# cv-core/MIT-Driverless-CV-TrainingInfra

Measured on AMD Instinct MI355X. Metric: images/sec training (YOLOv3 416^2 + RektNet 80^2), higher is better.
Workload: dtype bf16; 1 GPU; CVC-YOLOv3 yolo_baseline 416x416 classes=80, train step (fwd+bwd+Adam), 32 img/GPU; global_batch=32, parallelism=dp1, hipgraph=False, optimizer=FusedAdam

## Files before the change

include/mdcv_hip.h:

```cpp
#ifndef MDCV_HIP_H
#define MDCV_HIP_H
#ifdef __cplusplus
extern "C" {
#endif

#define MDCV_OK 0
#define MDCV_EARG (-1)
#define MDCV_F32 0
#define MDCV_BF16 1
#define MDCV_TUNED(dtype, code) (((dtype) & 0xff) | ((code) * 256))
#define MDCV_ACT_NONE 0
#define MDCV_ACT_LEAKY 1
#define MDCV_ACT_RELU 2

int mdcv_conv2d(int dtype, int mode, const void* in, int in_ldc, const void* w_packed, void* out, int out_ldc,
                const float* bias, const void* addsrc, int add_ldc, float* stats_partial,
                int B, int Hin, int Win, int Cin, int Hout, int Wout, int Nout,
                int KH, int KW, int stride, int pad, int dil, void* stream);
int mdcv_conv2d_affine_act(int dtype, const void* in, int in_ldc, const void* w_packed, void* out, int out_ldc, const float* scale,
                           const float* shift, const void* addsrc, int add_ldc, int act, float slope, int B, int Hin, int Win, int Cin,
                           int Hout, int Wout, int Nout, int KH, int KW, int stride, int pad, int dil, void* stream);
int mdcv_conv2d_dgrad_bnsums_rows(int dtype, int B, int Hin, int Win, int Cin, int Hout, int Wout, int Nout, int KH, int KW, int stride,
                                  int pad, int dil, int in_ldc);
int mdcv_conv2d_dgrad_bnsums(int dtype, const void* in, int in_ldc, const void* w_packed, void* out, int out_ldc, const void* addsrc,
                             int add_ldc, int B, int Hin, int Win, int Cin, int Hout, int Wout, int Nout, int KH, int KW, int stride,
                             int pad, int dil, const void* y, int ldy, const float* scale, const float* shift, const float* mean, int act,
                             float slope, float* partial, void* stream);
int mdcv_first_conv_ok(int dtype, int B, int H, int W, int Cin_pad, int Cout_pad, int KH, int KW, int stride, int pad, int dil, int ldx);
int mdcv_first_conv_rows(int B, int H);
int mdcv_first_conv_stats(int dtype, const void* x, int ldx, const void* w_packed, float* partial, int B, int H, int W, void* stream);
int mdcv_first_conv_bn_act(int dtype, const void* x, int ldx, const void* w_packed, const float* scale, const float* shift, int act, float slope,
                           void* y, int ldy, void* z, int ldz, int B, int H, int W, void* stream);
int mdcv_conv2d_dgrad_s2_form_ok(int dtype, int B, int Hin, int Win, int Cin, int Hout, int Wout, int Nout, int KH, int KW, int stride,
                                 int pad, int dil, int in_ldc);
int mdcv_xstats_words(int reps, int C);
int mdcv_xstats_reps(int rows, int C);
int mdcv_conv2d_xstats(int dtype, const void* in, int in_ldc, const void* w_packed, void* out, int out_ldc, const float* bias, void* xacc,
                       int reps, int B, int Hin, int Win, int Cin, int Hout, int Wout, int Nout, int KH, int KW, int stride, int pad, int dil,
                       void* stream);
int mdcv_pw_conv_fwd_xstats(int dtype, const void* y, int ldy, const float* scale, const float* shift, const void* resid, int ldr, int act,
                            float slope, void* z_out, int ldz, const void* w_packed, const float* bias, void* out, int out_ldc, void* xacc,
                            int reps, long long M, int K, int N, void* stream);
int mdcv_bn_act_fwd_xstats(int dtype, const void* y, int ldy, const void* xacc, int reps, double count, const float* gamma, const float* beta,
                           float* running_mean, float* running_var, float momentum, float eps, float* scale, float* shift, float* mean,
                           float* invstd, const void* resid, int ldr, void* out, int ldo, int M, int C, int act, float slope, void* stream);
int mdcv_conv2d_stats_rows(int M);
int mdcv_conv2d_stats_rows_geom(int dtype, int B, int Hout, int Wout, int Cin, int Nout, int KH, int KW, int stride, int pad, int dil,
                                int in_ldc);

int mdcv_conv2d_wgrad_splits(int dtype, int M, int Cout, int Ktot);
int mdcv_conv2d_wgrad_splits_geom(int dtype, int B, int Hin, int Win, int Cin, int Hout, int Wout, int Cout, int KH, int KW, int stride,
                                  int pad, int dil, int dy_ldc, int x_ldc);
int mdcv_conv2d_wgrad(int dtype, const void* dy, int dy_ldc, const void* x, int x_ldc, float* ws, int splits,
                      float* dw_oihw, int accumulate, int B, int Hin, int Win, int Cin, int Cin_real,
                      int Hout, int Wout, int Cout, int Cout_real, int KH, int KW, int stride, int pad, int dil, void* stream);

int mdcv_pack_weights(int dtype, const float* w_oihw, void* w_fwd, void* w_dgrad, int Cout, int Cin, int KH, int KW,
                      int Cout_pad, int Cin_pad, void* stream);

int mdcv_pack_weights_batched(int dtype, const void* table, int nlayers, int max_taps, void* stream);

int mdcv_nchw_to_nhwc(int dtype, const float* src, void* dst, int B, int C, int H, int W, int ldc, int Cpad, void* stream);
int mdcv_nhwc_to_nchw(int dtype, const void* src, int ldc, float* dst, int B, int C, int H, int W, void* stream);

int mdcv_partial_reduce(const float* partial, int rows, int nsums, int C, double* accum, void* stream);
int mdcv_bn_finalize(double* accum, double count, const float* gamma, const float* beta, float* running_mean, float* running_var,
                     float momentum, float eps, float* scale, float* shift, float* mean, float* invstd, int C, void* stream);
int mdcv_bn_eval_coeffs(const float* gamma, const float* beta, const float* running_mean, const float* running_var, float eps,
                        float* scale, float* shift, int C, void* stream);
int mdcv_bn_eval_coeffs_bias(const float* gamma, const float* beta, const float* running_mean, const float* running_var, float eps,
                             const float* conv_bias, float* scale, float* shift, int C, void* stream);
int mdcv_bn_act_fwd(int dtype, const void* y1, int ld1, const float* s1, const float* b1, const void* y2, int ld2, const float* s2,
                    const float* b2, const void* resid, int ldr, void* out, int ldo, int M, int C, int act, float slope, void* stream);
int mdcv_bn_act_bwd_reduce_ws_floats(int dtype, int M, int C, int nsums);
int mdcv_bn_stats_finalize(const float* partial, int rows, double* accum, double count, const float* gamma, const float* beta,
                           float* running_mean, float* running_var, float momentum, float eps, float* scale, float* shift, float* mean,
                           float* invstd, int C, void* stream);
int mdcv_bn_act_bwd_reduce_finalize(int dtype, const void* dout, int ldd, const void* y1, int ld1, const float* s1, const float* b1,
                                    const float* mean1, const float* invstd1, const void* y2, int ld2, const float* s2, const float* b2,
                                    const float* mean2, const float* invstd2, float* partial_ws, int M, int C, int act, float slope,
                                    double count, const float* gamma1, float* dgamma1, float* dbeta1, float* cA1, float* cB1, float* cC1,
                                    const float* gamma2, float* dgamma2, float* dbeta2, float* cA2, float* cB2, float* cC2, void* stream);
int mdcv_bn_bwd_finalize_rows(const float* partial, int rows, int C, double count, const float* gamma, const float* mean,
                              const float* invstd, float* dgamma, float* dbeta, float* cA, float* cB, float* cC, void* stream);
int mdcv_bn_act_bwd_reduce(int dtype, const void* dout, int ldd, const void* y1, int ld1, const float* s1, const float* b1,
                           const float* mean1, const float* invstd1, const void* y2, int ld2, const float* s2, const float* b2,
                           const float* mean2, const float* invstd2, double* accum, float* partial_ws, int M, int C, int act, float slope,
                           void* stream);
int mdcv_bn_bwd_finalize(double* accum, int kx, int nsums, int zero_after, double count, const float* gamma, const float* mean,
                         const float* invstd, float* dgamma, float* dbeta, float* cA, float* cB, float* cC, int C, void* stream);
int mdcv_bn_act_bwd_apply(int dtype, const void* dout, int ldd, const void* y1, int ld1, const float* s1, const float* b1,
                          const float* cA1, const float* cB1, const float* cC1, void* dy1, int ldy1,
                          const void* y2, int ld2, const float* s2, const float* b2, const float* cA2, const float* cB2,
                          const float* cC2, void* dy2, int ldy2, int M, int C, int act, float slope, void* stream);
int mdcv_colsum(int dtype, const void* x, int ldc, int M, int C, double* accum, void* stream);
int mdcv_colsum_ws_floats(int dtype, int M, int C);
int mdcv_colsum_f32(int dtype, const void* x, int ldc, int M, int C, float* partial_ws, float* out, void* stream);
int mdcv_accum_to_f32(double* accum, float* out, int n, int zero_after, void* stream);

int mdcv_upsample2x_fwd(int dtype, const void* in, int ldi, void* out, int ldo, int B, int H, int W, int C, void* stream);
int mdcv_upsample2x_bwd(int dtype, const void* dout, int ldo, void* din, int ldi, int B, int H, int W, int C, void* stream);

int mdcv_maxpool2x2_fwd(int dtype, const void* in, int ldi, void* out, int ldo, unsigned char* idx, int B, int H, int W, int C, int stride,
                        void* stream);
int mdcv_maxpool2x2_bwd(int dtype, const void* dout, int ldo, const unsigned char* idx, void* din, int ldi, int B, int H, int W, int C, int stride,
                        void* stream);

int mdcv_maxpool_fwd(int dtype, const void* in, int ldi, void* out, int ldo, unsigned char* idx, int B, int H, int W, int C, int k, int stride,
                     int pad, void* stream);
int mdcv_maxpool_bwd(int dtype, const void* dout, int ldo, const unsigned char* idx, void* din, int ldi, int B, int H, int W, int C, int k, int stride,
                     int pad, void* stream);
int mdcv_upsample_fwd(int dtype, const void* in, int ldi, void* out, int ldo, int B, int H, int W, int C, int scale, void* stream);
int mdcv_upsample_bwd(int dtype, const void* dout, int ldo, void* din, int ldi, int B, int H, int W, int C, int scale, void* stream);

long long mdcv_yolo_head_workspace_bytes(int B, int A, int Gh, int Gw);
int mdcv_yolo_head_train(int dtype, const void* logits, int ldc, void* dlogits, int ldd, int Cpad, const float* targets,
                         const float* anchors_scaled, int B, int T, int A, int C, int Gh, int Gw, float thresh, float xy_loss,
                         float wh_loss, float obj_loss, float noobj_loss, void* workspace, float* out7, const float* gscale,
                         void* stream);
int mdcv_yolo_head_grad(int dtype, const void* logits, int ldc, void* dlogits, int ldd, int Cpad, const float* targets,
                        const float* anchors_scaled, int B, int T, int A, int C, int Gh, int Gw, float thresh, float xy_loss,
                        float wh_loss, float obj_loss, float noobj_loss, void* workspace, const float* gscale, void* stream);
int mdcv_yolo_head_decode(int dtype, const void* logits, int ldc, const float* anchors_scaled, float stride, int B, int A, int C, int Gh,
                          int Gw, float* out, int rows_total, int row_off, void* stream);
int mdcv_bbox_iou(const float* box1, long long n1, int stride1, const float* box2, long long n2, int stride2, int corners, float* out, void* stream);
long long mdcv_build_targets_workspace_bytes(int B, int T, int A, int Gh, int Gw);
int mdcv_build_targets(const float* targets, const float* anchors, int B, int T, int A, int C, int Gh, int Gw, float thresh,
                       unsigned char* mask, unsigned char* conf_mask, float* tx, float* ty, float* tw, float* th, float* tconf,
                       unsigned char* tcls, void* workspace, int* err_out, void* stream);

int mdcv_head1x1_f32(const void* x_bf16, int ldx, const float* w, const float* bias, float* out, long long M, int C, int K, void* stream);
int mdcv_softargmax_fwd(int dtype, const void* logits, int ldc, int B, int K, int H, int W, float* hm, float* pts, void* stream);
int mdcv_softargmax_bwd(int dtype, const float* hm, const float* pts, const float* dpts, const float* dhm, float* sdot_ws, int B, int K,
                        int H, int W, void* dlogits, int ldd, void* stream);
int mdcv_cross_ratio_loss(const float* hm, const float* pts, const float* thm, const float* tpts, int B, int H, int W, int loss_type,
                          int include_geo, float gamma_horz, float gamma_vert, double* acc_ws, const float* gscale, float* out3,
                          float* dpts, float* dhm, void* stream);

#define MDCV_KPT_EVAL_ROW 12
int mdcv_kpt_eval_rows(const float* hm, const float* pts, const float* thm, const float* tpts, int B, int H, int W, int loss_type, int include_geo,
                       float gamma_horz, float gamma_vert, float dist_sx, float dist_sy, float* rows, void* stream);

#define MDCV_NMS_MAX_TOPK 512
long long mdcv_nms_workspace_bytes(int n);
int mdcv_nms(const float* boxes, const float* scores, int n, float overlap, int top_k, long long* keep, int* count, void* workspace,
             void* stream);
long long mdcv_detect_post_workspace_bytes(int B, int N);
int mdcv_detect_post(const float* pred, int B, int N, int C, const float* targets, int T, float conf_thres, float nms_thres,
                     float iou_thres, float width, float height, int top_k, float* out_boxes, float* out_prob, int* out_cls,
                     long long* out_index, unsigned char* out_correct, int* out_count, float* out_stats, void* workspace,
                     void* stream);
int mdcv_average_precision(const unsigned char* tp, const float* conf, int m, int n_gt, float* out3, void* stream);

int mdcv_crop_resize(const float* frames, int B, int C, int H, int W, const float* boxes, const int* count, int K, float scale_x,
                     float scale_y, float off_x, float off_y, int out_h, int out_w, float* out, int* owner, int* total, void* stream);

int mdcv_crop_resize_u8(const unsigned char* frames, int B, int C, int H, int W, const float* boxes, const int* count, int K, float scale_x,
                        float scale_y, float off_x, float off_y, int out_h, int out_w, float* out, int* owner, int* total, void* stream);

int mdcv_synth_cone_batch(unsigned int seed, int step, int B, int T, int H, int W, int num_classes, float* images, float* targets, void* stream);
int mdcv_synth_crop_batch(unsigned int seed, int step, int B, int size, float* images, float* heatmaps, float* points, void* stream);

#define MDCV_IMGLOAD_DESC 20
long long mdcv_imgload_workspace_bytes(int B, int max_scr_w, int max_scr_h);
int mdcv_imgload_batch(const int* desc_host, const int* desc, int B, const int* coefs, long long n_coefs, const unsigned char* src,
                       long long src_bytes, int max_scr_w, int max_scr_h, int C, int H, int W, void* workspace, float* out, void* stream);

#define MDCV_IMGAUG_DESC 24
long long mdcv_imgaug_workspace_bytes(int B, int H, int W);
int mdcv_imgload_aug_batch(const int* desc_host, const int* desc, const int* aug_host, const int* aug, int B, const int* coefs, long long n_coefs,
                           const unsigned char* src, long long src_bytes, int max_scr_w, int max_scr_h, int C, int H, int W, void* workspace,
                           void* aug_workspace, float* out, void* stream);

#define MDCV_IMGLOAD_FREF 4
int mdcv_imgload_frames_batch(const int* desc_host, const int* desc, const long long* fref_host, const long long* fref, int B, const int* coefs,
                              long long n_coefs, const unsigned char* src, long long src_bytes, const unsigned char* pool, long long pool_bytes,
                              int max_scr_w, int max_scr_h, int C, int H, int W, void* workspace, float* out, void* stream);
int mdcv_imgload_aug_frames_batch(const int* desc_host, const int* desc, const long long* fref_host, const long long* fref, const int* aug_host,
                                  const int* aug, int B, const int* coefs, long long n_coefs, const unsigned char* src, long long src_bytes,
                                  const unsigned char* pool, long long pool_bytes, int max_scr_w, int max_scr_h, int C, int H, int W,
                                  void* workspace, void* aug_workspace, float* out, void* stream);

#define MDCV_IMGFX_DESC 24
int mdcv_imgfx_batch(const int* fx_host, const int* fx, int B, const unsigned char* luts, int n_luts, int C, int H, int W, const float* src,
                     float* dst, void* stream);

#define MDCV_KPTLOAD_DESC 20
#define MDCV_KPTLOAD_MIN_SIZE 16
#define MDCV_KPTLOAD_MAX_SIZE 256
#define MDCV_KPTLOAD_MAX_SIDE 4096
int mdcv_kptload_batch(const int* desc_host, const int* desc, int B, const unsigned char* src, long long src_bytes, int S, float* images,
                       float* heatmaps, void* stream);

#define MDCV_DETECT_DESC 6
int mdcv_detect_draw_boxes(const long long* desc_host, const long long* desc, int B, const float* boxes, const int* count, int K,
                           unsigned char* pool, long long pool_bytes, int red, int green, int blue, double* frame_boxes, int* rects,
                           int* skipped, void* stream);

int mdcv_detect_map_boxes(const long long* desc_host, const long long* desc, int B, const float* boxes, const int* count, int K,
                          long long pool_bytes, double* frame_boxes, int* rects, int* skipped, void* stream);

int mdcv_crop_resize_frames_u8(const long long* desc_host, const long long* desc, int B, const unsigned char* pool, long long pool_bytes,
                               const int* rects, const int* count, int K, int max_per_frame, int S, float* crops, int* owner, int* window,
                               int* total, void* stream);
int mdcv_kpt_draw_points(const long long* desc_host, const long long* desc, int n_images, unsigned char* pool, long long pool_bytes,
                         const float* pts, const int* window, const int* owner, int M, const unsigned char* colours, int* centers,
                         int* skipped, void* stream);
int mdcv_kpt_heatmap_mosaic(const float* hm, int B, int S, unsigned char* out, void* stream);

int mdcv_adam_step(float* params, const float* grads, float* exp_avg, float* exp_avg_sq, long long n, int step, float lr, float beta1,
                   float beta2, float eps, float weight_decay, float grad_scale, void* stream);
int mdcv_sgd_step(float* params, const float* grads, float* momentum_buf, long long n, int step, float lr, float momentum, float weight_decay,
                  float grad_scale, void* stream);

int mdcv_device_info(int* cu_count, int* wave_size, long long* hbm_bytes, char* arch, int arch_len);
int mdcv_event_create(void** ev);
int mdcv_event_record(void* ev, void* stream);
int mdcv_event_sync(void* ev);
int mdcv_event_elapsed_ms(void* start, void* stop, float* ms);
int mdcv_event_destroy(void* ev);
int mdcv_probe_mfma(int blocks, int iters, float* sink, double* flops, void* stream);
int mdcv_stream_fork(void* from, void* to, int device_scope);
int mdcv_stream_fork_arm(void* from, int device_scope, void** ev_out);
int mdcv_stream_fork_wait(void* to, void* ev);
int mdcv_profile_begin(void);
int mdcv_profile_count(void);
int mdcv_profile_stop(void);
int mdcv_profile_read(int i, float* ms, char* name, int name_len);
int mdcv_graph_begin(void* stream);
int mdcv_graph_end(void* stream, void** graph_exec);
int mdcv_graph_launch(void* graph_exec, void* stream);
int mdcv_graph_destroy(void* graph_exec);

int mdcv_pw_rows(long long M, int K);
int mdcv_pw_conv_fwd(int dtype, const void* y, int ldy, const float* scale, const float* shift, const void* resid, int ldr, int act,
                     float slope, void* z_out, int ldz, const void* w_packed, const float* bias, void* out, int out_ldc,
                     float* stats_partial, long long M, int K, int N, void* stream);

int mdcv_pw_bwd_slabs(int dtype, long long M, int Cin, int Cout, int ldy, int ldx, int lddx, int ldadd, int ldfy);
int mdcv_pw_bwd(int dtype, const void* dy, int ldy, const void* x, int ldx, const void* wd_packed, void* dx, int lddx, const void* addsrc,
                int ldadd, float* ws, int slabs, const void* fy, int ldfy, const float* fscale, const float* fshift, const float* fmean, int fact,
                float fslope, float* fpartial, long long M, int Cin, int Cout, void* stream);
int mdcv_conv2d_wgrad_bnapply_ok(int dtype, int B, int Hin, int Win, int Cin, int Hout, int Wout, int Cout, int KH, int KW, int stride,
                                 int pad, int dil, int dz_ldc, int y_ldc, int x_ldc);
int mdcv_conv2d_wgrad_bnapply(int dtype, const void* dz, int dz_ldc, const void* y, int y_ldc, const float* scale, const float* shift,
                              const float* cA, const float* cB, const float* cC, int act, float slope, const void* x, int x_ldc, float* ws,
                              int splits, float* dw_oihw, int accumulate, int B, int Hin, int Win, int Cin, int Cin_real, int Hout, int Wout,
                              int Cout, int Cout_real, int KH, int KW, int stride, int pad, int dil, void* stream);
int mdcv_wgrad_reduce(const float* ws, int splits, float* dw_oihw, int accumulate, int Cout_pad, int Cout, int Cin_pad, int Cin, int KK,
                      void* stream);

int mdcv_comm_unique_id(void* id128);
int mdcv_comm_init(void** comm, int nranks, const void* id128, int rank);
int mdcv_comm_allreduce_sum(void* comm, float* buf, long long n, void* stream);
int mdcv_comm_destroy(void* comm);

#ifdef __cplusplus
}
#endif
#endif
```

mit-driverless-cv-traininginfra_amd/csrc/conv_igemm.hip:

```cpp
#include "conv_gemm.h"
#include "conv_shift.h"
#include "wgrad_gemm.h"
#include "wgrad_shift.h"
#include "wgrad_stream.h"

extern "C" {

static int conv2d_impl(int dtype, int mode, const void* in, int in_ldc, const void* w_packed, void* out, int out_ldc,
                       const float* bias, const void* addsrc, int add_ldc, float* stats_partial,
                       int B, int Hin, int Win, int Cin, int Hout, int Wout, int Nout,
                       int KH, int KW, int stride, int pad, int dil, const BnFuseArgs* fuse, void* stream, const EpiArgs* epi = nullptr,
                       const XAccArgs* xacc = nullptr) {
  if (!in || !w_packed || !out) return MDCV_EARG;
  if (xacc && (mode != 0 || stats_partial || fuse || epi || !xacc->acc || xacc->reps < 1 || (xacc->reps & (xacc->reps - 1)))) return MDCV_EARG;
  if (epi && (mode != 0 || stats_partial || fuse)) return MDCV_EARG;
  if ((Cin & 7) || (Nout & 7) || (in_ldc & 7) || (out_ldc & 7) || (addsrc && (add_ldc & 7))) return MDCV_EARG;
  if (stride != 1 && stride != 2) return MDCV_EARG;
  if (mode != 0 && mode != 1) return MDCV_EARG;
  ConvArgs a;
  a.in = in; a.w = w_packed; a.out = out; a.bias = bias; a.addsrc = addsrc; a.stats = stats_partial;
  a.in_ldc = in_ldc; a.out_ldc = out_ldc; a.add_ldc = add_ldc;
  a.Hin = Hin; a.Win = Win; a.Cin = Cin; a.Hout = Hout; a.Wout = Wout; a.Nout = Nout;
  a.KH = KH; a.KW = KW; a.stride = stride; a.pad = pad; a.dil = dil;
  a.M = B * Hout * Wout; a.Ktot = KH * KW * Cin; a.tiles_n = 0; a.sshift = stride == 2 ? 1 : 0; a.tiles_total = 0; a.xcd_chunk = 0;
  a.ph = a.pw = a.kh0 = a.kw0 = 0; a.Hs = Hout; a.Ws = Wout; a.nkh = KH; a.nkw = KW; a.cls_split = 0;
  a.fuse = fuse ? *fuse : BnFuseArgs{};
  a.epi = epi ? *epi : EpiArgs{nullptr, 0, 0.f};
  a.xacc = xacc ? *xacc : XAccArgs{nullptr, 1};
  if (a.M <= 0) return MDCV_OK;
  hipStream_t st = (hipStream_t)stream;
  const int es = dtype == MDCV_BF16 ? 2 : 4;
  const bool small = conv_operands_small((long long)B * Hin * Win * in_ldc * es, (long long)Nout * KH * KW * Cin * es);
  if (mode == 1 && stride == 2 && dil == 1 && small && (TUNE().conv_variant != 0 || fuse)) {
    if (!bias && KH == 3 && KW == 3 && pad == 1 && Hout == 2 * Hin && Wout == 2 * Win && TUNE().conv_variant < 0 &&
        mdcv_shift_s2_dgrad_eligible(dtype, B, Hin, Win, Cin, Nout, in_ldc))
      return mdcv_shift_conv(3, in, in_ldc, w_packed, out, out_ldc, nullptr, addsrc, add_ldc, nullptr, B, Hin, Win, Cin, Nout, fuse, st, nullptr, 1);
    if (TUNE().conv_s2_allcls && dtype == MDCV_BF16 && KH == 3 && KW == 3 && pad == 1 && !(Hout & 1) && !(Wout & 1) && (Cin % 32) == 0 && TUNE().conv_deep_s2 &&
        TUNE().conv_tall_s2) {
      ConvArgs c = a;
      c.Hs = Hout / 2; c.Ws = Wout / 2;
      c.M = B * c.Hs * c.Ws;
      c.fuse.row_base = 0;
      const int rc = mdcv_cd_bf16_s2_all(c, st, B);
      if (rc != MDCV_EARG) return rc;
    }
    int row_base = 0;
    for (int cls = 0; cls < 4; ++cls) {
      ConvArgs c = a;
      c.ph = cls >> 1; c.pw = cls & 1;
      c.Hs = (Hout - c.ph + 1) / 2; c.Ws = (Wout - c.pw + 1) / 2;
      c.kh0 = (c.ph + pad) & 1; c.kw0 = (c.pw + pad) & 1;
      c.nkh = (KH - c.kh0 + 1) / 2; c.nkw = (KW - c.kw0 + 1) / 2;
      c.M = B * c.Hs * c.Ws;
      c.Ktot = c.nkh * c.nkw * Cin;
      if (c.M <= 0) continue;
      c.fuse.row_base = row_base;
      row_base += cdiv(c.M, 128);
      int rc;
      if (c.nkh <= 0 || c.nkw <= 0) { c.nkh = c.nkh > 0 ? c.nkh : 0; c.nkw = c.nkw > 0 ? c.nkw : 0; c.Ktot = 0; }
      if (dtype == MDCV_BF16) rc = mdcv_cd_bf16_s2(c, st, B);
      else if (dtype == MDCV_F32) rc = mdcv_cd_f32_s2(c, st, B);
      else return MDCV_EARG;
      if (rc) return rc;
    }
    return MDCV_OK;
  }
  const bool shift_ok = Hin == Hout && Win == Wout && mdcv_shift_eligible(dtype, B, Hout, Wout, Cin, Nout, KH, KW, stride, pad, dil, in_ldc);
  if (shift_ok && (TUNE().conv_variant < 0 || fuse))
    return mdcv_shift_conv(mode, in, in_ldc, w_packed, out, out_ldc, bias, addsrc, add_ldc, stats_partial, B, Hout, Wout, Cin, Nout, fuse, st, epi, dil, xacc);
  if (fuse) {
    if (!small) return MDCV_EARG;
    MdcvTune t2 = TUNE();
    if (t2.conv_variant >= 0 && t2.conv_variant < 6) t2.conv_variant = -1;
    const TuneScope lds_dma_only(t2);
    return dtype == MDCV_BF16 ? mdcv_cd_bf16_dgrad(a, st, B) : (dtype == MDCV_F32 ? mdcv_cd_f32_dgrad(a, st, B) : MDCV_EARG);
  }
  if (shift_ok && stats_partial) {
    const int r0 = cdiv(a.M, 128), r1 = mdcv_shift_fwd_stats_rows(B, Hout, Wout, Nout, dil);
    if (r1 > r0) {
      hipError_t e = hipMemsetAsync(stats_partial + (size_t)r0 * 2 * Nout, 0, (size_t)(r1 - r0) * 2 * Nout * sizeof(float), st);
      if (e != hipSuccess) return (int)e;
    }
  }
  if (dtype == MDCV_BF16) return mode == 0 ? mdcv_cd_bf16_fwd(a, st, B) : mdcv_cd_bf16_dgrad(a, st, B);
  if (dtype == MDCV_F32) return mode == 0 ? mdcv_cd_f32_fwd(a, st, B) : mdcv_cd_f32_dgrad(a, st, B);
  return MDCV_EARG;
}

int mdcv_conv2d(int dtype, int mode, const void* in, int in_ldc, const void* w_packed, void* out, int out_ldc,
                const float* bias, const void* addsrc, int add_ldc, float* stats_partial,
                int B, int Hin, int Win, int Cin, int Hout, int Wout, int Nout,
                int KH, int KW, int stride, int pad, int dil, void* stream) {
  MDCV_TUNE_ENTRY(dtype, MDCV_TUNE_CONV);
  return conv2d_impl(dtype, mode, in, in_ldc, w_packed, out, out_ldc, bias, addsrc, add_ldc, stats_partial, B, Hin, Win, Cin, Hout, Wout, Nout,
                     KH, KW, stride, pad, dil, nullptr, stream);
}

int mdcv_xstats_words(int reps, int C) { return reps * XACC_DIGITS * 2 * C; }
int mdcv_conv2d_xstats(int dtype, const void* in, int in_ldc, const void* w_packed, void* out, int out_ldc, const float* bias, void* xacc,
                       int reps, int B, int Hin, int Win, int Cin, int Hout, int Wout, int Nout, int KH, int KW, int stride, int pad, int dil,
                       void* stream) {
  MDCV_TUNE_ENTRY(dtype, MDCV_TUNE_CONV);
  const XAccArgs x{reinterpret_cast<long long*>(xacc), reps};
  return conv2d_impl(dtype, 0, in, in_ldc, w_packed, out, out_ldc, bias, nullptr, 0, nullptr, B, Hin, Win, Cin, Hout, Wout, Nout, KH, KW,
                     stride, pad, dil, nullptr, stream, nullptr, &x);
}

int mdcv_conv2d_affine_act(int dtype, const void* in, int in_ldc, const void* w_packed, void* out, int out_ldc, const float* scale,
                           const float* shift, const void* addsrc, int add_ldc, int act, float slope, int B, int Hin, int Win, int Cin,
                           int Hout, int Wout, int Nout, int KH, int KW, int stride, int pad, int dil, void* stream) {
  MDCV_TUNE_ENTRY(dtype, MDCV_TUNE_CONV);
  if (act < 0 || act > 2) return MDCV_EARG;
  const EpiArgs e{scale, act, slope};
  return conv2d_impl(dtype, 0, in, in_ldc, w_packed, out, out_ldc, shift, addsrc, add_ldc, nullptr, B, Hin, Win, Cin, Hout, Wout, Nout,
                     KH, KW, stride, pad, dil, nullptr, stream, &e);
}

int mdcv_conv2d_dgrad_bnsums_rows(int dtype, int B, int Hin, int Win, int Cin, int Hout, int Wout, int Nout, int KH, int KW, int stride,
                                  int pad, int dil, int in_ldc) {
  MDCV_TUNE_ENTRY(dtype, MDCV_TUNE_CONV);
  const int es = 2;
  if (dtype != MDCV_BF16) return 0;
  if (!conv_operands_small((long long)B * Hin * Win * in_ldc * es, (long long)Nout * KH * KW * Cin * es)) return 0;
  if (Hin == Hout && Win == Wout && mdcv_shift_eligible(dtype, B, Hout, Wout, Cin, Nout, KH, KW, stride, pad, dil, in_ldc))
    return mdcv_shift_stats_rows(B, Hout, Wout, dil, Nout);
  if (stride == 2 && dil == 1 && KH == 3 && KW == 3 && pad == 1 && Hout == 2 * Hin && Wout == 2 * Win && TUNE().conv_variant < 0 &&
      mdcv_shift_s2_dgrad_eligible(dtype, B, Hin, Win, Cin, Nout, in_ldc))
    return mdcv_shift_s2_rows(B, Hin, Win);
  if (stride == 2 && dil == 1) {
    int rows = 0;
    for (int cls = 0; cls < 4; ++cls) {
      const int ph = cls >> 1, pw = cls & 1;
      const int m = B * ((Hout - ph + 1) / 2) * ((Wout - pw + 1) / 2);
      if (m > 0) rows += cdiv(m, 128);
    }
    return rows;
  }
  return cdiv(B * Hout * Wout, 128);
}

int mdcv_conv2d_dgrad_bnsums(int dtype, const void* in, int in_ldc, const void* w_packed, void* out, int out_ldc, const void* addsrc,
                             int add_ldc, int B, int Hin, int Win, int Cin, int Hout, int Wout, int Nout, int KH, int KW, int stride,
                             int pad, int dil, const void* y, int ldy, const float* scale, const float* shift, const float* mean, int act,
                             float slope, float* partial, void* stream) {
  MDCV_TUNE_ENTRY(dtype, MDCV_TUNE_CONV);
  if (!y || !scale || !shift || !mean || !partial || (ldy & 7)) return MDCV_EARG;
  if (mdcv_conv2d_dgrad_bnsums_rows(dtype, B, Hin, Win, Cin, Hout, Wout, Nout, KH, KW, stride, pad, dil, in_ldc) <= 0) return MDCV_EARG;
  BnFuseArgs f;
  f.y = y; f.scale = scale; f.shift = shift; f.mean = mean; f.partial = partial; f.ldy = ldy; f.act = act; f.row_base = 0;
  f.slope = act == 2 ? 0.f : slope;
  return conv2d_impl(dtype, 1, in, in_ldc, w_packed, out, out_ldc, nullptr, addsrc, add_ldc, nullptr, B, Hin, Win, Cin, Hout, Wout, Nout,
                     KH, KW, stride, pad, dil, &f, stream);
}

int mdcv_conv2d_dgrad_s2_form_ok(int dtype, int B, int Hin, int Win, int Cin, int Hout, int Wout, int Nout, int KH, int KW, int stride,
                                 int pad, int dil, int in_ldc) {
  MDCV_TUNE_ENTRY(dtype, MDCV_TUNE_CONV);
  return dtype == MDCV_BF16 && stride == 2 && dil == 1 && KH == 3 && KW == 3 && pad == 1 && Hout == 2 * Hin && Wout == 2 * Win &&
         TUNE().conv_variant < 0 && (long long)B * Hin * Win * in_ldc * 2 < (1LL << 31) &&
         mdcv_shift_s2_dgrad_eligible(dtype, B, Hin, Win, Cin, Nout, in_ldc);
}

int mdcv_conv2d_stats_rows(int M) { return cdiv(M, 128); }
int mdcv_conv2d_stats_rows_geom(int dtype, int B, int Hout, int Wout, int Cin, int Nout, int KH, int KW, int stride, int pad, int dil,
                                int in_ldc) {
  MDCV_TUNE_ENTRY(dtype, MDCV_TUNE_CONV);
  if (mdcv_shift_eligible(dtype, B, Hout, Wout, Cin, Nout, KH, KW, stride, pad, dil, in_ldc)) return mdcv_shift_fwd_stats_rows(B, Hout, Wout, Nout, dil);
  return cdiv(B * Hout * Wout, 128);
}

int mdcv_conv2d_wgrad_splits(int dtype, int M, int Cout, int Ktot) {
  MDCV_TUNE_ENTRY(dtype, MDCV_TUNE_WGRAD);
  const int bp = dtype == MDCV_BF16 ? 128 : 64;
  const int tiles = cdiv(Cout, 128) * cdiv(Ktot, 128);
  const int slots = TUNE().wgrad_slots;
  int s = slots / tiles;
  const int max_s = cdiv(M, bp * 4);
  if (s > max_s) s = max_s;
  if (s < 1) s = 1;
  int pps = cdiv(cdiv(M, s), bp) * bp;
  return cdiv(M, pps);
}

enum WgradFamily { WG_STEM, WG_STREAM, WG_SHIFT, WG_S2, WG_GENERIC };

static bool wgrad_eligible(WgradFamily f, const WgradGeom& g) {
  const int v = TUNE().wgrad_variant;
  if (f == WG_GENERIC) return true;
  if (v == 9 || (v == 10 && f != WG_SHIFT)) return false;
  const bool same = g.Hin == g.Hout && g.Win == g.Wout;
  switch (f) {
    case WG_STEM:
      return same && mdcv_wgrad_stem_eligible(g.dtype, g.B, g.Hout, g.Wout, g.Cin, g.Cout, g.KH, g.KW, g.stride, g.pad, g.dil, g.dy_ldc, g.x_ldc);
    case WG_STREAM:
      return same && mdcv_wgrad_stream_eligible(g.dtype, g.B, g.Hout, g.Wout, g.Cin, g.Cout, g.KH, g.KW, g.stride, g.pad, g.dil, g.dy_ldc, g.x_ldc);
    case WG_S2:
      return mdcv_wgrad_s2_eligible(g.dtype, g.B, g.Hin, g.Win, g.Cin, g.Hout, g.Wout, g.Cout, g.KH, g.KW, g.stride, g.pad, g.dil, g.dy_ldc, g.x_ldc);
    default: break;
  }
  if (!same || !mdcv_wgrad_shift_eligible(g.dtype, g.B, g.Hout, g.Wout, g.Cin, g.Cout, g.KH, g.KW, g.stride, g.pad, g.dil, g.dy_ldc, g.x_ldc)) return false;
  if (v == 8) return true;
  const long long Mq = (long long)g.B * (g.Hout + 1) * (g.Wout + 1);
  const int s = mdcv_wgrad_shift_splits(g.B, g.Hout, g.Wout, g.Cin, g.Cout);
  if (Mq / (64LL * s) >= 128) return true;
  return v == 11 && mdcv_conv2d_wgrad_splits(g.dtype, g.B * g.Hout * g.Wout, g.Cout, g.KH * g.KW * g.Cin) == 1;
}

static int wgrad_family_splits(WgradFamily f, const WgradGeom& g) {
  switch (f) {
    case WG_STEM:   return mdcv_wgrad_stem_splits(g.B, g.Hout, g.Wout);
    case WG_STREAM: return mdcv_wgrad_stream_splits(g.B, g.Hout, g.Wout, g.Cin, g.Cout, g.dil);
    case WG_SHIFT:  return mdcv_wgrad_shift_splits(g.B, g.Hout, g.Wout, g.Cin, g.Cout);
    case WG_S2:     return mdcv_wgrad_s2_splits(g.B, g.Hout, g.Wout, g.Cin, g.Cout);
    default:        return mdcv_conv2d_wgrad_splits(g.dtype, g.B * g.Hout * g.Wout, g.Cout, g.KH * g.KW * g.Cin);
  }
}

static bool wgrad_family_splits_ok(WgradFamily f, const WgradGeom& g, int splits) {
  switch (f) {
    case WG_STEM:   return mdcv_wgrad_stem_splits_ok(splits, g.B, g.Hout, g.Wout);
    case WG_STREAM: return mdcv_wgrad_stream_splits_ok(splits, g.B, g.Hout, g.Wout, g.Cin, g.Cout, g.dil);
    case WG_SHIFT:  return mdcv_wgrad_shift_splits_ok(splits, g.B, g.Hout, g.Wout);
    case WG_S2:     return mdcv_wgrad_s2_splits_ok(splits, g.B, g.Hout, g.Wout);
    default:        return true;
  }
}

static WgradFamily choose_wgrad_family(const WgradGeom& g, int splits) {
  for (int f = WG_STEM; f < WG_GENERIC; ++f)
    if (wgrad_eligible((WgradFamily)f, g) && (splits == 0 || wgrad_family_splits_ok((WgradFamily)f, g, splits))) return (WgradFamily)f;
  return WG_GENERIC;
}

int mdcv_conv2d_wgrad_splits_geom(int dtype, int B, int Hin, int Win, int Cin, int Hout, int Wout, int Cout, int KH, int KW, int stride,
                                  int pad, int dil, int dy_ldc, int x_ldc) {
  MDCV_TUNE_ENTRY(dtype, MDCV_TUNE_WGRAD);
  const WgradGeom g{dtype, B, Hin, Win, Cin, Hout, Wout, Cout, KH, KW, stride, pad, dil, dy_ldc, x_ldc};
  return wgrad_family_splits(choose_wgrad_family(g, 0), g);
}

int mdcv_conv2d_wgrad(int dtype, const void* dy, int dy_ldc, const void* x, int x_ldc, float* ws, int splits,
                      float* dw_oihw, int accumulate, int B, int Hin, int Win, int Cin, int Cin_real,
                      int Hout, int Wout, int Cout, int Cout_real, int KH, int KW, int stride, int pad, int dil, void* stream) {
  MDCV_TUNE_ENTRY(dtype, MDCV_TUNE_WGRAD);
  if (!dy || !x || !ws || !dw_oihw) return MDCV_EARG;
  if ((Cin & 7) || (Cout & 7) || (dy_ldc & 7) || (x_ldc & 7) || splits < 1) return MDCV_EARG;
  const WgradGeom g{dtype, B, Hin, Win, Cin, Hout, Wout, Cout, KH, KW, stride, pad, dil, dy_ldc, x_ldc};
  hipStream_t st = (hipStream_t)stream;
  int rc, KK = 9, wrote_dw = 0;
  switch (choose_wgrad_family(g, splits)) {
    case WG_STEM:   KK = 49; rc = mdcv_wgrad_stem(dy, dy_ldc, x, x_ldc, ws, splits, B, Hout, Wout, st); break;
    case WG_STREAM: rc = mdcv_wgrad_stream(dy, dy_ldc, x, x_ldc, ws, splits, B, Hout, Wout, Cin, Cout, dil, st, dw_oihw, Cin_real, Cout_real, accumulate,
                                           &wrote_dw); break;
    case WG_SHIFT:  rc = mdcv_wgrad_shift(dy, dy_ldc, x, x_ldc, ws, splits, B, Hout, Wout, Cin, Cout, st); break;
    case WG_S2:     rc = mdcv_wgrad_s2(dy, dy_ldc, x, x_ldc, ws, splits, B, Hout, Wout, Cin, Cout, st); break;
    default:        KK = KH * KW; rc = launch_wgrad_gemm(g, dy, x, ws, splits, st); break;
  }
  if (rc || wrote_dw) return rc;
  return launch_wgrad_reduce(ws, dw_oihw, splits, Cout, Cout_real, Cin, Cin_real, KK, accumulate, st);
}

int mdcv_conv2d_wgrad_bnapply_ok(int dtype, int B, int Hin, int Win, int Cin, int Hout, int Wout, int Cout, int KH, int KW, int stride,
                                 int pad, int dil, int dz_ldc, int y_ldc, int x_ldc) {
  MDCV_TUNE_ENTRY(dtype, MDCV_TUNE_WGRAD);
  if (dtype != MDCV_BF16 || Cout > 32 || (Cin & 7) || (Cout & 7) || (dz_ldc & 7) || (y_ldc & 7) || (x_ldc & 7) || TUNE().wgrad_variant != 0) return 0;
  const WgradGeom g{dtype, B, Hin, Win, Cin, Hout, Wout, Cout, KH, KW, stride, pad, dil, dz_ldc, x_ldc};
  if (choose_wgrad_family(g, 0) != WG_GENERIC) return 0;
  const long long M = (long long)B * Hout * Wout;
  const int ldmax = dz_ldc > y_ldc ? dz_ldc : y_ldc;
  return M * ldmax * 2 < (1LL << 31) && (long long)B * Hin * Win * x_ldc * 2 < (1LL << 31) && TUNE().conv_variant != 0 &&
         (long long)B * Hin * Win + 256 < (1LL << 24) && M + 256 < (1 << 24) && Wout >= 8 && x_ldc < (1 << 23) && ldmax < (1 << 23);
}
int mdcv_conv2d_wgrad_bnapply(int dtype, const void* dz, int dz_ldc, const void* y, int y_ldc, const float* scale, const float* shift,
                              const float* cA, const float* cB, const float* cC, int act, float slope, const void* x, int x_ldc, float* ws,
                              int splits, float* dw_oihw, int accumulate, int B, int Hin, int Win, int Cin, int Cin_real, int Hout, int Wout,
                              int Cout, int Cout_real, int KH, int KW, int stride, int pad, int dil, void* stream) {
  MDCV_TUNE_ENTRY(dtype, MDCV_TUNE_WGRAD);
  if (!dz || !y || !scale || !shift || !cA || !cB || !cC || !x || !ws || !dw_oihw || splits < 1) return MDCV_EARG;
  if (!mdcv_conv2d_wgrad_bnapply_ok(dtype, B, Hin, Win, Cin, Hout, Wout, Cout, KH, KW, stride, pad, dil, dz_ldc, y_ldc, x_ldc)) return MDCV_EARG;
  const WgradGeom g{dtype, B, Hin, Win, Cin, Hout, Wout, Cout, KH, KW, stride, pad, dil, dz_ldc, x_ldc};
  const int rc = launch_wgrad_gemm_bnapply(g, dz, y, y_ldc, scale, shift, cA, cB, cC, act, slope, Cout_real, x, ws, splits, (hipStream_t)stream);
  if (rc) return rc;
  return launch_wgrad_reduce(ws, dw_oihw, splits, Cout, Cout_real, Cin, Cin_real, KH * KW, accumulate, (hipStream_t)stream);
}

}
```

mit-driverless-cv-traininginfra_amd/csrc/first_conv.hip:

```cpp
#include "common.h"

namespace {

constexpr int NW = 4;
constexpr int TR = 4;
constexpr int COUT = 32, CIN = 8, PXB = CIN * 2;

struct FirstConvArgs {
  const bf16_t* x; const bf16_t* wf;
  bf16_t* y; bf16_t* z; const float* scale; const float* shift;
  float* partial;
  int ldx, ldy, ldz, B, H, W, strips, act;
  float slope;
};

template <int MODE>
__global__ __launch_bounds__(NW * 64) void first_conv_kernel(FirstConvArgs a) {
  extern __shared__ __attribute__((aligned(16))) unsigned char smem[];
  const int tid = threadIdx.x, lane = tid & 63, wave = tid >> 6;
  const int l16 = lane & 15, kg = lane >> 4;
  const int img = blockIdx.x / a.strips, strip = blockIdx.x - img * a.strips;
  const int r0 = strip * TR;
  const int WP = a.W + 2;
  unsigned char* const stage = smem + (size_t)(TR + 2) * (WP + 16) * PXB;
  {
    const bf16_t* xi = a.x + (size_t)img * a.H * a.W * a.ldx;
    const int total = (TR + 2) * WP;
    for (int base = tid; base < total; base += 8 * NW * 64) {
      uint4 v[8];
#pragma unroll
      for (int u = 0; u < 8; ++u) {
        const int i = base + u * NW * 64;
        int rr = 0;
#pragma unroll
        for (int k = 1; k < TR + 2; ++k) rr += i >= k * WP;
        const int cc = i - rr * WP;
        const int gy = r0 - 1 + rr, gx = cc - 1;
        v[u] = make_uint4(0u, 0u, 0u, 0u);
        if (i < total && gy >= 0 && gy < a.H && gx >= 0 && gx < a.W) v[u] = *reinterpret_cast<const uint4*>(xi + ((size_t)gy * a.W + gx) * a.ldx);
      }
#pragma unroll
      for (int u = 0; u < 8; ++u) {
        const int i = base + u * NW * 64;
        if (i < total) *reinterpret_cast<uint4*>(smem + (size_t)i * PXB) = v[u];
      }
    }
  }
  bf16x8_t wa[2][3];
#pragma unroll
  for (int h = 0; h < 2; ++h)
#pragma unroll
    for (int s = 0; s < 3; ++s) {
      const int tap = 4 * s + kg;
      uint4 v = make_uint4(0u, 0u, 0u, 0u);
      if (tap < 9) v = *reinterpret_cast<const uint4*>(a.wf + ((size_t)(h * 16 + l16) * 9 + tap) * CIN);
      wa[h][s] = __builtin_bit_cast(bf16x8_t, v);
    }
  int boff[3];
#pragma unroll
  for (int s = 0; s < 3; ++s) {
    int tap = 4 * s + kg;
    tap = tap < 9 ? tap : 8;
    const int dy = tap / 3, dx = tap - dy * 3;
    boff[s] = (dy * WP + l16 + dx) * PXB;
  }
  float sc[2][4], sh[2][4];
  if constexpr (MODE == 1) {
#pragma unroll
    for (int h = 0; h < 2; ++h)
#pragma unroll
      for (int r = 0; r < 4; ++r) { sc[h][r] = a.scale[h * 16 + kg * 4 + r]; sh[h][r] = a.shift[h * 16 + kg * 4 + r]; }
  }
  float ssum[2][4], ssq[2][4];
#pragma unroll
  for (int h = 0; h < 2; ++h)
#pragma unroll
    for (int r = 0; r < 4; ++r) { ssum[h][r] = 0.f; ssq[h][r] = 0.f; }
  __syncthreads();

  unsigned char* const st = stage + wave * 2048;
  for (int lr = wave; lr < TR; lr += NW) {
    const int row = r0 + lr;
    if (row >= a.H) break;
    const size_t rowpix = ((size_t)img * a.H + row) * a.W;
    const unsigned char* const rb = smem + (size_t)lr * WP * PXB;
    uint4 bn[3];
#pragma unroll
    for (int s = 0; s < 3; ++s) bn[s] = *reinterpret_cast<const uint4*>(rb + boff[s]);
    for (int c0 = 0; c0 < a.W; c0 += 16) {
      uint4 b[3];
#pragma unroll
      for (int s = 0; s < 3; ++s) b[s] = bn[s];
      if (c0 + 16 < a.W) {
#pragma unroll
        for (int s = 0; s < 3; ++s) bn[s] = *reinterpret_cast<const uint4*>(rb + boff[s] + (c0 + 16) * PXB);
      }
      f32x4_t acc[2] = {{0.f, 0.f, 0.f, 0.f}, {0.f, 0.f, 0.f, 0.f}};
#pragma unroll
      for (int s = 0; s < 3; ++s) {
        const bf16x8_t bb = __builtin_bit_cast(bf16x8_t, b[s]);
        acc[0] = __builtin_amdgcn_mfma_f32_16x16x32_bf16(wa[0][s], bb, acc[0], 0, 0, 0);
        acc[1] = __builtin_amdgcn_mfma_f32_16x16x32_bf16(wa[1][s], bb, acc[1], 0, 0, 0);
      }
      if constexpr (MODE == 0) {
        if (c0 + l16 < a.W) {
#pragma unroll
          for (int h = 0; h < 2; ++h)
#pragma unroll
            for (int r = 0; r < 4; ++r) { const float v = acc[h][r]; ssum[h][r] += v; ssq[h][r] += v * v; }
        }
      } else {
#pragma unroll
        for (int h = 0; h < 2; ++h) {
          uint2 yq, zq;
          yq.x = pack_bf16x2(acc[h][0], acc[h][1]); yq.y = pack_bf16x2(acc[h][2], acc[h][3]);
          float v[4];
          v[0] = __uint_as_float(yq.x << 16); v[1] = __uint_as_float(yq.x & 0xffff0000u);
          v[2] = __uint_as_float(yq.y << 16); v[3] = __uint_as_float(yq.y & 0xffff0000u);
#pragma unroll
          for (int r = 0; r < 4; ++r) {
            const float pre = __builtin_fmaf(v[r], sc[h][r], sh[h][r]);
            v[r] = a.act == 0 ? pre : (pre > 0.f ? pre : pre * a.slope);
          }
          zq.x = pack_bf16x2(v[0], v[1]); zq.y = pack_bf16x2(v[2], v[3]);
          *reinterpret_cast<uint2*>(st + l16 * 64 + (h * 16 + kg * 4) * 2) = yq;
          *reinterpret_cast<uint2*>(st + 1024 + l16 * 64 + (h * 16 + kg * 4) * 2) = zq;
        }
        asm volatile("s_waitcnt lgkmcnt(0)" ::: "memory");
        const uint4 yo = *reinterpret_cast<const uint4*>(st + lane * 16);
        const uint4 zo = *reinterpret_cast<const uint4*>(st + 1024 + lane * 16);
        asm volatile("s_waitcnt lgkmcnt(0)" ::: "memory");
        const int px = c0 + (lane >> 2);
        if (px < a.W) {
          *reinterpret_cast<uint4*>(a.y + (rowpix + px) * a.ldy + (lane & 3) * 8) = yo;
          *reinterpret_cast<uint4*>(a.z + (rowpix + px) * a.ldz + (lane & 3) * 8) = zo;
        }
      }
    }
  }
  if constexpr (MODE == 0) {
#pragma unroll
    for (int h = 0; h < 2; ++h)
#pragma unroll
      for (int r = 0; r < 4; ++r)
#pragma unroll
        for (int o = 8; o >= 1; o >>= 1) { ssum[h][r] += __shfl_xor(ssum[h][r], o, 64); ssq[h][r] += __shfl_xor(ssq[h][r], o, 64); }
    float* red = reinterpret_cast<float*>(stage);
    if (l16 == 0) {
#pragma unroll
      for (int h = 0; h < 2; ++h)
#pragma unroll
        for (int r = 0; r < 4; ++r) {
          red[(wave * 2 + 0) * COUT + h * 16 + kg * 4 + r] = ssum[h][r];
          red[(wave * 2 + 1) * COUT + h * 16 + kg * 4 + r] = ssq[h][r];
        }
    }
    __syncthreads();
    if (tid < 2 * COUT) {
      float t = 0.f;
#pragma unroll
      for (int w = 0; w < NW; ++w) t += red[w * 2 * COUT + tid];
      a.partial[(size_t)blockIdx.x * 2 * COUT + tid] = t;
    }
  }
}

static size_t lds_bytes(int W) { return (size_t)(TR + 2) * (W + 2 + 16) * PXB + NW * 2048; }
static int nstrips(int H) { return (H + TR - 1) / TR; }

}

extern "C" {

int mdcv_first_conv_ok(int dtype, int B, int H, int W, int Cin_pad, int Cout_pad, int KH, int KW, int stride, int pad, int dil, int ldx) {
  return (dtype & 0xff) == MDCV_BF16 && Cin_pad == CIN && ldx == CIN && Cout_pad == COUT && KH == 3 && KW == 3 && stride == 1 && pad == 1 && dil == 1 &&
         B >= 1 && H >= 1 && W >= 1 && W <= 1024 && (long long)B * H * W * COUT * 2 < (1LL << 40);
}
int mdcv_first_conv_rows(int B, int H) { return B * nstrips(H); }

int mdcv_first_conv_stats(int dtype, const void* x, int ldx, const void* w_packed, float* partial, int B, int H, int W, void* stream) {
  if (!x || !w_packed || !partial || !mdcv_first_conv_ok(dtype, B, H, W, CIN, COUT, 3, 3, 1, 1, 1, ldx)) return MDCV_EARG;
  FirstConvArgs a{};
  a.x = reinterpret_cast<const bf16_t*>(x); a.wf = reinterpret_cast<const bf16_t*>(w_packed); a.partial = partial;
  a.ldx = ldx; a.B = B; a.H = H; a.W = W; a.strips = nstrips(H);
  const int lds = (int)lds_bytes(W);
  static DynLds dyn;
  if (hipError_t e = mdcv_dyn_lds(dyn, reinterpret_cast<const void*>(first_conv_kernel<0>), lds); e != hipSuccess) return (int)e;
  MDCV_LAUNCH(first_conv_kernel<0>, dim3((unsigned)(B * a.strips)), dim3(NW * 64), lds, (hipStream_t)stream, a);
  MDCV_CHECK_LAUNCH();
  return MDCV_OK;
}

int mdcv_first_conv_bn_act(int dtype, const void* x, int ldx, const void* w_packed, const float* scale, const float* shift, int act, float slope,
                           void* y, int ldy, void* z, int ldz, int B, int H, int W, void* stream) {
  if (!x || !w_packed || !scale || !shift || !y || !z || (ldy & 7) || (ldz & 7) || ldy < COUT || ldz < COUT ||
      !mdcv_first_conv_ok(dtype, B, H, W, CIN, COUT, 3, 3, 1, 1, 1, ldx))
    return MDCV_EARG;
  FirstConvArgs a{};
  a.x = reinterpret_cast<const bf16_t*>(x); a.wf = reinterpret_cast<const bf16_t*>(w_packed);
  a.y = reinterpret_cast<bf16_t*>(y); a.z = reinterpret_cast<bf16_t*>(z); a.scale = scale; a.shift = shift;
  a.ldx = ldx; a.ldy = ldy; a.ldz = ldz; a.B = B; a.H = H; a.W = W; a.strips = nstrips(H); a.act = act; a.slope = act == 2 ? 0.f : slope;
  const int lds = (int)lds_bytes(W);
  static DynLds dyn;
  if (hipError_t e = mdcv_dyn_lds(dyn, reinterpret_cast<const void*>(first_conv_kernel<1>), lds); e != hipSuccess) return (int)e;
  MDCV_LAUNCH(first_conv_kernel<1>, dim3((unsigned)(B * a.strips)), dim3(NW * 64), lds, (hipStream_t)stream, a);
  MDCV_CHECK_LAUNCH();
  return MDCV_OK;
}

}
```

mit-driverless-cv-traininginfra_amd/csrc/wgrad_gemm.h:

```cpp
#pragma once
#include <hip/hip_runtime.h>

struct WgradGeom {
  int dtype, B, Hin, Win, Cin, Hout, Wout, Cout, KH, KW, stride, pad, dil;
  long long dy_ldc, x_ldc;
};

int launch_wgrad_gemm(const WgradGeom& g, const void* dy, const void* x, float* ws, int splits, hipStream_t st);
int launch_wgrad_gemm_bnapply(const WgradGeom& g, const void* dz, const void* y, int y_ldc, const float* scale, const float* shift, const float* cA,
                              const float* cB, const float* cC, int act, float slope, int Cout_real, const void* x, float* ws, int splits,
                              hipStream_t st);
int launch_wgrad_reduce(const float* ws, float* dw_oihw, int splits, int Cout_pad, int Cout_real, int Cin_pad, int Cin_real, int KK, int accumulate,
                        hipStream_t st);
```

mit-driverless-cv-traininginfra_amd/csrc/wgrad_gemm.hip:

```cpp
#include "conv_gemm.h"
#include "wgrad_gemm.h"

namespace {

struct WgradArgs {
  const void* dy; const void* x; float* ws;
  int dy_ldc, x_ldc;
  int Hin, Win, Cin, Hout, Wout, Cout;
  int KH, KW, stride, pad, dil;
  int M, Ktot, tiles_k, tiles_ck, pix_per_split, blocks_total, xcd_chunk;
  const void* y; int y_ldc, act, creal; float slope;
  const float* s1; const float* b1; const float* cA; const float* cB; const float* cC;
};

template <typename T>
__global__ __launch_bounds__(256) void conv_wgrad_kernel(WgradArgs a) {
  constexpr int VEC = ET<T>::VEC;
  constexpr int NP = 4;
  constexpr int BP = NP * 4 * VEC;
  constexpr int OQ = 128 / VEC;
  constexpr int PPP = 2 * (256 / OQ);
  constexpr int RB = 64 * NP + 16;
  constexpr int FM = 4, FN = 4;
  constexpr int OROW = 132;
  static_assert(PPP * NP == BP, "pass geometry");
  extern __shared__ __attribute__((aligned(16))) unsigned char smem[];
  const int logical = (int)(blockIdx.x & 7) * a.xcd_chunk + (int)(blockIdx.x >> 3);
  if (logical >= a.blocks_total) return;
  const int tid = threadIdx.x, lane = tid & 63, wave = tid >> 6;
  const int wm = wave >> 1, wn = wave & 1;
  const int split = logical / a.tiles_ck;
  const int tck = logical - split * a.tiles_ck;
  const int tile_co = tck / a.tiles_k, tile_k = tck - tile_co * a.tiles_k;
  const T* __restrict__ dy = reinterpret_cast<const T*>(a.dy);
  const T* __restrict__ x = reinterpret_cast<const T*>(a.x);

  const int oct = tid % OQ, pp = tid / OQ;
  const int co0 = tile_co * 128 + oct * VEC;
  const bool a_ok = co0 < a.Cout;
  const int kcol0 = tile_k * 128 + oct * VEC;
  const bool b_ok = kcol0 < a.Ktot;
  int dh, dw, ci;
  {
    const int kk = b_ok ? kcol0 : 0;
    const int tap = kk / a.Cin;
    ci = kk - tap * a.Cin;
    const int kh = tap / a.KW, kw = tap - kh * a.KW;
    dh = kh * a.dil - a.pad; dw = kw * a.dil - a.pad;
  }
  const int p_begin = split * a.pix_per_split;
  const int p_end = min(a.M, p_begin + a.pix_per_split);
  const int HWo = a.Hout * a.Wout;

  uint4 ra[2 * NP], rb[2 * NP];
  auto load_step = [&](int m0) {
#pragma unroll
    for (int ps = 0; ps < NP; ++ps) {
      const int m = m0 + ps * PPP + 2 * pp;
      int img = m / HWo, rem = m - img * HWo;
      int ho = rem / a.Wout, wo = rem - ho * a.Wout;
#pragma unroll
      for (int e = 0; e < 2; ++e) {
        const bool pv = m + e < p_end;
        uint4 va = make_uint4(0, 0, 0, 0), vb = make_uint4(0, 0, 0, 0);
        if (pv && a_ok) va = *reinterpret_cast<const uint4*>(dy + ((size_t)(m + e) * a.dy_ldc + co0));
        const int hi = ho * a.stride + dh, wi = wo * a.stride + dw;
        if (pv && b_ok && (unsigned)hi < (unsigned)a.Hin && (unsigned)wi < (unsigned)a.Win)
          vb = *reinterpret_cast<const uint4*>(x + ((size_t)((img * a.Hin + hi) * a.Win + wi) * a.x_ldc + ci));
        ra[2 * ps + e] = va; rb[2 * ps + e] = vb;
        if (++wo == a.Wout) { wo = 0; if (++ho == a.Hout) { ho = 0; ++img; } }
      }
    }
  };
  auto store_step = [&]() {
    unsigned char* sA = smem;
    unsigned char* sB = smem + 128 * RB;
#pragma unroll
    for (int ps = 0; ps < NP; ++ps) {
      const unsigned a0[4] = {ra[2 * ps].x, ra[2 * ps].y, ra[2 * ps].z, ra[2 * ps].w}, a1[4] = {ra[2 * ps + 1].x, ra[2 * ps + 1].y, ra[2 * ps + 1].z, ra[2 * ps + 1].w};
      const unsigned b0[4] = {rb[2 * ps].x, rb[2 * ps].y, rb[2 * ps].z, rb[2 * ps].w}, b1[4] = {rb[2 * ps + 1].x, rb[2 * ps + 1].y, rb[2 * ps + 1].z, rb[2 * ps + 1].w};
      if (sizeof(T) == 2) {
        const int cb = ps * 64 + pp * 4;
#pragma unroll
        for (int q = 0; q < 4; ++q) {
          *reinterpret_cast<unsigned*>(sA + ((2 * q) * OQ + oct) * RB + cb) = (a0[q] & 0xffffu) | (a1[q] << 16);
          *reinterpret_cast<unsigned*>(sA + ((2 * q + 1) * OQ + oct) * RB + cb) = (a0[q] >> 16) | (a1[q] & 0xffff0000u);
          *reinterpret_cast<unsigned*>(sB + ((2 * q) * OQ + oct) * RB + cb) = (b0[q] & 0xffffu) | (b1[q] << 16);
          *reinterpret_cast<unsigned*>(sB + ((2 * q + 1) * OQ + oct) * RB + cb) = (b0[q] >> 16) | (b1[q] & 0xffff0000u);
        }
      } else {
        const int cb = ps * 64 + pp * 8;
#pragma unroll
        for (int q = 0; q < 4; ++q) {
          *reinterpret_cast<uint2*>(sA + (q * OQ + oct) * RB + cb) = make_uint2(a0[q], a1[q]);
          *reinterpret_cast<uint2*>(sB + (q * OQ + oct) * RB + cb) = make_uint2(b0[q], b1[q]);
        }
      }
    }
  };

  f32x4_t acc[FM][FN];
#pragma unroll
  for (int i = 0; i < FM; ++i)
#pragma unroll
    for (int j = 0; j < FN; ++j) acc[i][j] = f32x4_t{0.f, 0.f, 0.f, 0.f};
  const int nt = (p_end - p_begin + BP - 1) / BP;
  if (nt > 0) {
    load_step(p_begin);
    store_step();
  }
  __syncthreads();
  for (int t = 0; t < nt; ++t) {
    if (t + 1 < nt) load_step(p_begin + (t + 1) * BP);
    Frag<T>::template mma<FM, FN, NP, RB>(smem + wm * 64 * RB, smem + 128 * RB + wn * 64 * RB, lane, acc);
    __syncthreads();
    if (t + 1 < nt) store_step();
    __syncthreads();
  }
  float* so = reinterpret_cast<float*>(smem);
#pragma unroll
  for (int i = 0; i < FM; ++i)
#pragma unroll
    for (int j = 0; j < FN; ++j)
#pragma unroll
      for (int r = 0; r < 4; ++r) {
        const int Ra = (wm * FM + i) * 16 + (lane >> 4) * 4 + r;
        const int Rb = (wn * FN + j) * 16 + (lane & 15);
        const int col = (Ra % OQ) * VEC + Ra / OQ;
        const int kl = (Rb % OQ) * VEC + Rb / OQ;
        so[col * OROW + kl] = acc[i][j][r];
      }
  __syncthreads();
  float* __restrict__ ws = a.ws + (size_t)split * a.Cout * a.Ktot;
  for (int v = tid; v < 128 * 32; v += 256) {
    const int row = v >> 5, c4 = (v & 31) * 4;
    const int co = tile_co * 128 + row, k = tile_k * 128 + c4;
    if (co < a.Cout && k < a.Ktot)
      *reinterpret_cast<float4*>(ws + (size_t)co * a.Ktot + k) = *reinterpret_cast<const float4*>(so + row * OROW + c4);
  }
}

__device__ __forceinline__ void fast_divmod(int n, int d, float inv, int& q, int& r) {
  q = (int)((float)n * inv);
  r = n - q * d;
  const int lt = r < 0;       q -= lt; r += lt ? d : 0;
  const int ge = r >= d;      q += ge; r -= ge ? d : 0;
}

typedef __attribute__((ext_vector_type(4))) short s16x4_t;
typedef __attribute__((address_space(3))) s16x4_t lds_s16x4_t;

template <int OFF> __device__ __forceinline__ s16x4_t lds_tr16_asm(unsigned addr) {
  s16x4_t v;
  asm volatile("ds_read_b64_tr_b16 %0, %1 offset:%2" : "=v"(v) : "v"(addr), "n"(OFF) : "memory");
  return v;
}
__device__ __forceinline__ unsigned lds_addr(const unsigned char* p) {
  return (unsigned)(size_t)(const __attribute__((address_space(3))) unsigned char*)p;
}
template <int N> __device__ __forceinline__ void wait_lds_tr(bf16x8_t& a0) { asm volatile("s_waitcnt lgkmcnt(%1)" : "+v"(a0) : "n"(N) : "memory"); }
template <int N> __device__ __forceinline__ void wait_lds_tr(bf16x8_t& a0, bf16x8_t& a1, bf16x8_t& b0) {
  asm volatile("s_waitcnt lgkmcnt(%3)" : "+v"(a0), "+v"(a1), "+v"(b0) : "n"(N) : "memory");
}
template <int N> __device__ __forceinline__ void wait_lds_tr(bf16x8_t& a0, bf16x8_t& a1, bf16x8_t& a2, bf16x8_t& a3, bf16x8_t& b0) {
  asm volatile("s_waitcnt lgkmcnt(%5)" : "+v"(a0), "+v"(a1), "+v"(a2), "+v"(a3), "+v"(b0) : "n"(N) : "memory");
}

template <int BP, int STAGES, bool SAME>
__global__ __launch_bounds__(256) void conv_wgrad_dma_kernel(WgradArgs a, unsigned dy_bytes, unsigned x_bytes) {
  constexpr int NJ = BP / 16;
  constexpr int GD = 2 * NJ;
  constexpr int TILE = BP * 256;
  constexpr int OROW = 132;
  constexpr unsigned OOB = 0x80000000u;
  extern __shared__ __attribute__((aligned(1024))) unsigned char smem[];
  const int logical = (int)(blockIdx.x & 7) * a.xcd_chunk + (int)(blockIdx.x >> 3);
  if (logical >= a.blocks_total) return;
  const int tid = threadIdx.x, lane = tid & 63;
  const int wave = __builtin_amdgcn_readfirstlane(tid >> 6);
  const int wm = wave >> 1, wn = wave & 1;
  const int split = logical / a.tiles_ck;
  const int tck = logical - split * a.tiles_ck;
  const int tile_co = tck / a.tiles_k, tile_k = tck - tile_co * a.tiles_k;
  const __amdgpu_buffer_rsrc_t rdy = __builtin_amdgcn_make_buffer_rsrc(const_cast<void*>(a.dy), 0, dy_bytes, 0x00020000);
  const __amdgpu_buffer_rsrc_t rx = __builtin_amdgcn_make_buffer_rsrc(const_cast<void*>(a.x), 0, x_bytes, 0x00020000);

  const int r = lane >> 4, q = lane & 15;
  const int lcol = q ^ (2 * (r + 4 * (wave & 1)));
  const int co0 = tile_co * 128 + lcol * 8;
  const bool a_ok = co0 < a.Cout;
  const int kcol0 = tile_k * 128 + lcol * 8;
  const bool b_ok = kcol0 < a.Ktot;
  int dh, dw, ci;
  {
    const int kk = b_ok ? kcol0 : 0;
    const int tap = kk / a.Cin;
    ci = kk - tap * a.Cin;
    const int kh = tap / a.KW, kw = tap - kh * a.KW;
    dh = kh * a.dil - a.pad; dw = kw * a.dil - a.pad;
  }
  const int p_begin = split * a.pix_per_split;
  const int p_end = min(a.M, p_begin + a.pix_per_split);
  const int HWo = a.Hout * a.Wout;
  const float inv_hw = 1.0f / (float)HWo, inv_w = 1.0f / (float)a.Wout;
  const unsigned ldy2 = (unsigned)a.dy_ldc * 2u, lx2 = (unsigned)a.x_ldc * 2u;
  const unsigned lane_a = (unsigned)co0 * 2u;
  const int lane_b = SAME ? ((dh * a.Win + dw) * a.x_ldc + ci) * 2 : ci * 2;
  const bool taps = a.KH * a.KW > 1 || a.pad != 0;

  auto issue = [&](int m0, int buf) {
    unsigned char* sA = smem + buf * 2 * TILE;
    unsigned char* sB = sA + TILE;
    int m = m0 + 4 * wave + r;
    int img = 0, ho = 0, wo = 0;
    if (!SAME || taps) {
      int rem;
      fast_divmod(m, HWo, inv_hw, img, rem);
      fast_divmod(rem, a.Wout, inv_w, ho, wo);
    }
#pragma unroll
    for (int j = 0; j < NJ; ++j) {
      const int chunk = wave + 4 * j;
      const bool pv = m < p_end;
      const unsigned offa = (pv & a_ok) ? __umul24((unsigned)m, ldy2) + lane_a : OOB;
      __builtin_amdgcn_raw_ptr_buffer_load_lds(rdy, (lds_void_t*)(sA + chunk * 1024), 16, offa, 0, 0, 0);
      unsigned offb;
      bool ok = pv & b_ok;
      if (SAME) {
        if (taps) ok = ok & ((unsigned)(ho + dh) < (unsigned)a.Hin) & ((unsigned)(wo + dw) < (unsigned)a.Win);
        offb = __umul24((unsigned)m, lx2) + (unsigned)lane_b;
      } else {
        const int hi = ho * a.stride + dh, wi = wo * a.stride + dw;
        ok = ok & ((unsigned)hi < (unsigned)a.Hin) & ((unsigned)wi < (unsigned)a.Win);
        offb = __umul24((unsigned)((img * a.Hin + hi) * a.Win + wi), lx2) + (unsigned)lane_b;
      }
      __builtin_amdgcn_raw_ptr_buffer_load_lds(rx, (lds_void_t*)(sB + chunk * 1024), 16, ok ? offb : OOB, 0, 0, 0);
      if (j + 1 < NJ) {
        m += 16;
        if (!SAME || taps) {
          wo += 16;
          int c = wo >= a.Wout; wo -= c ? a.Wout : 0; ho += c;
          c = wo >= a.Wout;     wo -= c ? a.Wout : 0; ho += c;
          c = ho >= a.Hout;     ho -= c ? a.Hout : 0; img += c;
        }
      }
    }
  };

  const int t = lane & 15, kq = lane >> 4;
  const int prow = kq * 4 + (t >> 2);
  const int sub = (t & 1) * 8;
  const int qlo = (t & 3) >> 1;
  const int g0 = 2 * (prow & 7);
  auto frag = [&](const unsigned char* tile, int ks, int F) -> bf16x8_t {
    const int row0 = ks * 32 + prow;
    const int c = 2 * F + qlo;
    const unsigned ad = lds_addr(tile) + (unsigned)(row0 * 256 + ((c ^ g0) << 4) + sub);
    const s16x4_t lo = lds_tr16_asm<0>(ad);
    const s16x4_t hi = lds_tr16_asm<16 * 256>(ad);
    typedef __attribute__((ext_vector_type(8))) short s16x8_t;
    const s16x8_t v = {lo[0], lo[1], lo[2], lo[3], hi[0], hi[1], hi[2], hi[3]};
    return __builtin_bit_cast(bf16x8_t, v);
  };

  f32x4_t acc[4][4];
#pragma unroll
  for (int i = 0; i < 4; ++i)
#pragma unroll
    for (int j = 0; j < 4; ++j) acc[i][j] = f32x4_t{0.f, 0.f, 0.f, 0.f};
  const int nt = (p_end - p_begin + BP - 1) / BP;
  auto compute = [&](int slot) {
    const unsigned char* sA = smem + slot * 2 * TILE;
    const unsigned char* sB = sA + TILE;
#pragma unroll
    for (int ks = 0; ks < BP / 32; ++ks) {
      bf16x8_t fa[4], fb[4];
#pragma unroll
      for (int i = 0; i < 4; ++i) fa[i] = frag(sA, ks, wm * 4 + i);
#pragma unroll
      for (int j = 0; j < 4; ++j) fb[j] = frag(sB, ks, wn * 4 + j);
      wait_lds_tr<6>(fa[0], fa[1], fa[2], fa[3], fb[0]);
#pragma unroll
      for (int i = 0; i < 4; ++i) acc[i][0] = __builtin_amdgcn_mfma_f32_16x16x32_bf16(fa[i], fb[0], acc[i][0], 0, 0, 0);
      wait_lds_tr<4>(fb[1]);
#pragma unroll
      for (int i = 0; i < 4; ++i) acc[i][1] = __builtin_amdgcn_mfma_f32_16x16x32_bf16(fa[i], fb[1], acc[i][1], 0, 0, 0);
      wait_lds_tr<2>(fb[2]);
#pragma unroll
      for (int i = 0; i < 4; ++i) acc[i][2] = __builtin_amdgcn_mfma_f32_16x16x32_bf16(fa[i], fb[2], acc[i][2], 0, 0, 0);
      wait_lds_tr<0>(fb[3]);
#pragma unroll
      for (int i = 0; i < 4; ++i) acc[i][3] = __builtin_amdgcn_mfma_f32_16x16x32_bf16(fa[i], fb[3], acc[i][3], 0, 0, 0);
    }
  };
  if (STAGES == 2) {
    if (nt > 0) issue(p_begin, 0);
    __syncthreads();
    for (int st = 0; st < nt; ++st) {
      const int cur = st & 1;
      if (st + 1 < nt) issue(p_begin + (st + 1) * BP, cur ^ 1);
      compute(cur);
      __syncthreads();
    }
  } else {
    int issued = 0;
    for (; issued < STAGES - 1 && issued < nt; ++issued) issue(p_begin + issued * BP, issued);
    int slot = 0, islot = issued % STAGES;
    for (int st = 0; st < nt; ++st) {
      const int newer = issued - 1 - st;
      if (newer >= STAGES - 2) asm volatile("s_waitcnt vmcnt(%0)" ::"n"(GD * (STAGES - 2)) : "memory");
      else if (newer == 1 && STAGES > 3) asm volatile("s_waitcnt vmcnt(%0)" ::"n"(GD) : "memory");
      else asm volatile("s_waitcnt vmcnt(0)" ::: "memory");
      __builtin_amdgcn_s_barrier();
      if (issued < nt) {
        issue(p_begin + issued * BP, islot);
        ++issued;
        islot = islot + 1 == STAGES ? 0 : islot + 1;
      }
      compute(slot);
      slot = slot + 1 == STAGES ? 0 : slot + 1;
    }
    __syncthreads();
  }
  float* so = reinterpret_cast<float*>(smem);
#pragma unroll
  for (int i = 0; i < 4; ++i)
#pragma unroll
    for (int j = 0; j < 4; ++j)
#pragma unroll
      for (int rr = 0; rr < 4; ++rr)
        so[((wm * 4 + i) * 16 + (lane >> 4) * 4 + rr) * OROW + (wn * 4 + j) * 16 + (lane & 15)] = acc[i][j][rr];
  __syncthreads();
  float* __restrict__ ws = a.ws + (size_t)split * a.Cout * a.Ktot;
  for (int v = tid; v < 128 * 32; v += 256) {
    const int row = v >> 5, c4 = (v & 31) * 4;
    const int co = tile_co * 128 + row, k = tile_k * 128 + c4;
    if (co < a.Cout && k < a.Ktot)
      *reinterpret_cast<float4*>(ws + (size_t)co * a.Ktot + k) = *reinterpret_cast<const float4*>(so + row * OROW + c4);
  }
}

template <bool SAME, int STAGES, bool BNA = false>
__global__ __launch_bounds__(256) void conv_wgrad_dma_narrow_kernel(WgradArgs a, unsigned dy_bytes, unsigned x_bytes) {
  constexpr int BP = 64, NJ = 4, GD = BNA ? 6 : 5;
  constexpr int TA = BP * 64 * (BNA ? 2 : 1), TB = BP * 256;
  constexpr int OROW = 132;
  constexpr unsigned OOB = 0x80000000u;
  extern __shared__ __attribute__((aligned(1024))) unsigned char smem[];
  const int logical = (int)(blockIdx.x & 7) * a.xcd_chunk + (int)(blockIdx.x >> 3);
  if (logical >= a.blocks_total) return;
  const int tid = threadIdx.x, lane = tid & 63;
  const int wave = __builtin_amdgcn_readfirstlane(tid >> 6);
  const int split = logical / a.tiles_ck;
  const int tile_k = logical - split * a.tiles_ck;
  const __amdgpu_buffer_rsrc_t rdy = __builtin_amdgcn_make_buffer_rsrc(const_cast<void*>(a.dy), 0, dy_bytes, 0x00020000);
  const __amdgpu_buffer_rsrc_t rx = __builtin_amdgcn_make_buffer_rsrc(const_cast<void*>(a.x), 0, x_bytes, 0x00020000);
  const __amdgpu_buffer_rsrc_t ry = __builtin_amdgcn_make_buffer_rsrc(const_cast<void*>(BNA ? a.y : a.dy), 0,
                                                                      BNA ? (unsigned)a.M * (unsigned)a.y_ldc * 2u : 0u, 0x00020000);

  const int ra = lane >> 2;
  const int coA = ((lane & 3) ^ (2 * ((ra >> 2) & 1))) * 8;
  const bool a_ok = coA < a.Cout;
  const int r = lane >> 4, q = lane & 15;
  const int lcol = q ^ (2 * (r + 4 * (wave & 1)));
  const int kcol0 = tile_k * 128 + lcol * 8;
  const bool b_ok = kcol0 < a.Ktot;
  int dh, dw, ci;
  {
    const int kk = b_ok ? kcol0 : 0;
    const int tap = kk / a.Cin;
    ci = kk - tap * a.Cin;
    const int kh = tap / a.KW, kw = tap - kh * a.KW;
    dh = kh * a.dil - a.pad; dw = kw * a.dil - a.pad;
  }
  const int p_begin = split * a.pix_per_split;
  const int p_end = min(a.M, p_begin + a.pix_per_split);
  const int HWo = a.Hout * a.Wout;
  const float inv_hw = 1.0f / (float)HWo, inv_w = 1.0f / (float)a.Wout;
  const unsigned ldy2 = (unsigned)a.dy_ldc * 2u, lx2 = (unsigned)a.x_ldc * 2u;
  const int lane_b = SAME ? ((dh * a.Win + dw) * a.x_ldc + ci) * 2 : ci * 2;
  const bool taps = a.KH * a.KW > 1 || a.pad != 0;

  auto issue = [&](int m0, int buf) {
    unsigned char* sA = smem + buf * (TA + TB);
    unsigned char* sB = sA + TA;
    {
      const int m = m0 + 16 * wave + ra;
      const unsigned offa = (m < p_end && a_ok) ? __umul24((unsigned)m, ldy2) + (unsigned)coA * 2u : OOB;
      __builtin_amdgcn_raw_ptr_buffer_load_lds(rdy, (lds_void_t*)(sA + wave * 1024), 16, offa, 0, 0, 0);
      if constexpr (BNA) {
        const unsigned offy = (m < p_end && a_ok) ? __umul24((unsigned)m, (unsigned)a.y_ldc * 2u) + (unsigned)coA * 2u : OOB;
        __builtin_amdgcn_raw_ptr_buffer_load_lds(ry, (lds_void_t*)(sA + BP * 64 + wave * 1024), 16, offy, 0, 0, 0);
      }
    }
    int m = m0 + 4 * wave + r;
    int img = 0, ho = 0, wo = 0;
    if (!SAME || taps) {
      int rem;
      fast_divmod(m, HWo, inv_hw, img, rem);
      fast_divmod(rem, a.Wout, inv_w, ho, wo);
    }
#pragma unroll
    for (int j = 0; j < NJ; ++j) {
      const int chunk = wave + 4 * j;
      bool ok = (m < p_end) & b_ok;
      unsigned offb;
      if (SAME) {
        if (taps) ok = ok & ((unsigned)(ho + dh) < (unsigned)a.Hin) & ((unsigned)(wo + dw) < (unsigned)a.Win);
        offb = __umul24((unsigned)m, lx2) + (unsigned)lane_b;
      } else {
        const int hi = ho * a.stride + dh, wi = wo * a.stride + dw;
        ok = ok & ((unsigned)hi < (unsigned)a.Hin) & ((unsigned)wi < (unsigned)a.Win);
        offb = __umul24((unsigned)((img * a.Hin + hi) * a.Win + wi), lx2) + (unsigned)lane_b;
      }
      __builtin_amdgcn_raw_ptr_buffer_load_lds(rx, (lds_void_t*)(sB + chunk * 1024), 16, ok ? offb : OOB, 0, 0, 0);
      if (j + 1 < NJ) {
        m += 16;
        if (!SAME || taps) {
          wo += 16;
          int c = wo >= a.Wout; wo -= c ? a.Wout : 0; ho += c;
          c = wo >= a.Wout;     wo -= c ? a.Wout : 0; ho += c;
          c = ho >= a.Hout;     ho -= c ? a.Hout : 0; img += c;
        }
      }
    }
  };

  const int t = lane & 15, kq = lane >> 4;
  const int prow = kq * 4 + (t >> 2);
  const int sub = (t & 1) * 8, qlo = (t & 3) >> 1;
  const int g0 = 2 * (prow & 7);
  typedef __attribute__((ext_vector_type(8))) short s16x8_t;
  auto fragB = [&](const unsigned char* tile, int ks, int F) -> bf16x8_t {
    const int row0 = ks * 32 + prow, c = 2 * F + qlo;
    const unsigned ad = lds_addr(tile) + (unsigned)(row0 * 256 + ((c ^ g0) << 4) + sub);
    const s16x4_t lo = lds_tr16_asm<0>(ad);
    const s16x4_t hi = lds_tr16_asm<16 * 256>(ad);
    const s16x8_t v = {lo[0], lo[1], lo[2], lo[3], hi[0], hi[1], hi[2], hi[3]};
    return __builtin_bit_cast(bf16x8_t, v);
  };
  auto fragA = [&](const unsigned char* tile, int ks, int F) -> bf16x8_t {
    const int row0 = ks * 32 + prow;
    const int col = (F ^ (kq & 1)) * 32 + (t & 3) * 8;
    const unsigned ad = lds_addr(tile) + (unsigned)(row0 * 64 + col);
    const s16x4_t lo = lds_tr16_asm<0>(ad);
    const s16x4_t hi = lds_tr16_asm<16 * 64>(ad);
    const s16x8_t v = {lo[0], lo[1], lo[2], lo[3], hi[0], hi[1], hi[2], hi[3]};
    return __builtin_bit_cast(bf16x8_t, v);
  };

  const int rowT = tid >> 2, coT = ((tid & 3) ^ (2 * ((rowT >> 2) & 1))) * 8;
  float ts1[BNA ? 8 : 1], tb1[BNA ? 8 : 1], tA[BNA ? 8 : 1], tB[BNA ? 8 : 1], tC[BNA ? 8 : 1];
  if constexpr (BNA) {
#pragma unroll
    for (int e = 0; e < 8; ++e) {
      const bool ok = coT + e < a.creal;
      ts1[e] = ok ? a.s1[coT + e] : 0.f; tb1[e] = ok ? a.b1[coT + e] : 0.f;
      tA[e] = ok ? a.cA[coT + e] : 0.f; tB[e] = ok ? a.cB[coT + e] : 0.f; tC[e] = ok ? a.cC[coT + e] : 0.f;
    }
  }
  auto transform = [&](int slot, int m0) {
    unsigned char* sA = smem + slot * (TA + TB);
    const unsigned ad = lds_addr(sA) + (unsigned)(tid * 16);
    typedef unsigned u32x4_t __attribute__((ext_vector_type(4)));
    u32x4_t rd, ry4;
    asm volatile("ds_read_b128 %0, %1" : "=v"(rd) : "v"(ad) : "memory");
    asm volatile("ds_read_b128 %0, %1 offset:4096" : "=v"(ry4) : "v"(ad) : "memory");
    asm volatile("s_waitcnt lgkmcnt(0)" : "+v"(rd), "+v"(ry4)::"memory");
    float d[8], v[8], o[8];
    ET<bf16_t>::unpack(make_uint4(rd[0], rd[1], rd[2], rd[3]), d);
    ET<bf16_t>::unpack(make_uint4(ry4[0], ry4[1], ry4[2], ry4[3]), v);
    const bool live = m0 + rowT < p_end;
#pragma unroll
    for (int e = 0; e < 8; ++e) o[e] = live ? mdcv_bn_bwd_dy(d[e], v[e], ts1[e], tb1[e], tA[e], tB[e], tC[e], a.act, a.slope) : 0.f;
    const uint4 qo = ET<bf16_t>::pack(o);
    const u32x4_t wo = {qo.x, qo.y, qo.z, qo.w};
    asm volatile("ds_write_b128 %0, %1" ::"v"(ad), "v"(wo) : "memory");
  };

  f32x4_t acc[2][2];
#pragma unroll
  for (int i = 0; i < 2; ++i)
#pragma unroll
    for (int j = 0; j < 2; ++j) acc[i][j] = f32x4_t{0.f, 0.f, 0.f, 0.f};
  const int nt = (p_end - p_begin + BP - 1) / BP;
  auto compute = [&](int slot) {
    const unsigned char* sA = smem + slot * (TA + TB);
    const unsigned char* sB = sA + TA;
#pragma unroll
    for (int ks = 0; ks < 2; ++ks) {
      bf16x8_t fa[2], fb[2];
#pragma unroll
      for (int i = 0; i < 2; ++i) fa[i] = fragA(sA, ks, i);
#pragma unroll
      for (int j = 0; j < 2; ++j) fb[j] = fragB(sB, ks, wave * 2 + j);
      wait_lds_tr<2>(fa[0], fa[1], fb[0]);
#pragma unroll
      for (int i = 0; i < 2; ++i) acc[i][0] = __builtin_amdgcn_mfma_f32_16x16x32_bf16(fa[i], fb[0], acc[i][0], 0, 0, 0);
      wait_lds_tr<0>(fb[1]);
#pragma unroll
      for (int i = 0; i < 2; ++i) acc[i][1] = __builtin_amdgcn_mfma_f32_16x16x32_bf16(fa[i], fb[1], acc[i][1], 0, 0, 0);
    }
  };
  int issued = 0;
  for (; issued < STAGES - 1 && issued < nt; ++issued) issue(p_begin + issued * BP, issued);
  int slot = 0, islot = issued % STAGES;
  for (int st = 0; st < nt; ++st) {
    const int newer = issued - 1 - st;
    if (newer >= 3 && STAGES >= 5) asm volatile("s_waitcnt vmcnt(%0)" ::"n"(GD * 3) : "memory");
    else if (newer >= 2 && STAGES >= 4) asm volatile("s_waitcnt vmcnt(%0)" ::"n"(GD * 2) : "memory");
    else if (newer >= 1 && STAGES >= 3) asm volatile("s_waitcnt vmcnt(%0)" ::"n"(GD) : "memory");
    else asm volatile("s_waitcnt vmcnt(0)" ::: "memory");
    __builtin_amdgcn_s_barrier();
    if (issued < nt) {
      issue(p_begin + issued * BP, islot);
      ++issued;
      islot = islot + 1 == STAGES ? 0 : islot + 1;
    }
    if constexpr (BNA) {
      transform(slot, p_begin + st * BP);
      asm volatile("s_waitcnt lgkmcnt(0)" ::: "memory");
      __builtin_amdgcn_s_barrier();
    }
    compute(slot);
    slot = slot + 1 == STAGES ? 0 : slot + 1;
  }
  __syncthreads();
  float* so = reinterpret_cast<float*>(smem);
#pragma unroll
  for (int i = 0; i < 2; ++i)
#pragma unroll
    for (int j = 0; j < 2; ++j)
#pragma unroll
      for (int rr = 0; rr < 4; ++rr)
        so[(i * 16 + (lane >> 4) * 4 + rr) * OROW + (wave * 2 + j) * 16 + (lane & 15)] = acc[i][j][rr];
  __syncthreads();
  float* __restrict__ ws = a.ws + (size_t)split * a.Cout * a.Ktot;
  for (int v = tid; v < 32 * 32; v += 256) {
    const int row = v >> 5, c4 = (v & 31) * 4;
    const int k = tile_k * 128 + c4;
    if (row < a.Cout && k < a.Ktot)
      *reinterpret_cast<float4*>(ws + (size_t)row * a.Ktot + k) = *reinterpret_cast<const float4*>(so + row * OROW + c4);
  }
}


template <int BP, int STAGES, bool SAME>
static int launch_wgrad_dma_t(const WgradArgs& a, unsigned grid, hipStream_t st, unsigned dyb, unsigned xb) {
  constexpr int RING = STAGES * 2 * BP * 256, EPI = 128 * 132 * 4;
  constexpr int LDS = RING > EPI ? RING : EPI;
  static DynLds dyn_lds;
  auto kern = conv_wgrad_dma_kernel<BP, STAGES, SAME>;
  if (hipError_t e = mdcv_dyn_lds(dyn_lds, reinterpret_cast<const void*>(kern), LDS); e != hipSuccess) return (int)e;
  MDCV_LAUNCH(kern, dim3(grid), dim3(256), LDS, st, a, dyb, xb);
  MDCV_CHECK_LAUNCH();
  return MDCV_OK;
}
template <bool SAME, int STAGES, bool BNA = false>
static int launch_wgrad_narrow_t(const WgradArgs& a, unsigned grid, hipStream_t st, unsigned dyb, unsigned xb) {
  constexpr int LDS = STAGES * (64 * 64 * (BNA ? 2 : 1) + 64 * 256);
  static DynLds dyn_lds;
  auto kern = conv_wgrad_dma_narrow_kernel<SAME, STAGES, BNA>;
  if (hipError_t e = mdcv_dyn_lds(dyn_lds, reinterpret_cast<const void*>(kern), LDS); e != hipSuccess) return (int)e;
  MDCV_LAUNCH(kern, dim3(grid), dim3(256), LDS, st, a, dyb, xb);
  MDCV_CHECK_LAUNCH();
  return MDCV_OK;
}
static int launch_wgrad_dma(const WgradArgs& a, unsigned grid, hipStream_t st, unsigned dyb, unsigned xb) {
  const bool same = a.stride == 1 && a.Hin == a.Hout && a.Win == a.Wout;
  if (a.Cout <= 32 && TUNE().wgrad_variant != 5)
    return same ? launch_wgrad_narrow_t<true, 4>(a, grid, st, dyb, xb) : launch_wgrad_narrow_t<false, 4>(a, grid, st, dyb, xb);
  if (TUNE().wgrad_variant == 4) return launch_wgrad_dma_t<64, 2, false>(a, grid, st, dyb, xb);
  return same ? launch_wgrad_dma_t<64, 2, true>(a, grid, st, dyb, xb) : launch_wgrad_dma_t<64, 2, false>(a, grid, st, dyb, xb);
}

bool fill_wgrad_args(WgradArgs& a, const WgradGeom& g, const void* dy, const void* x, float* ws, int splits, int bp) {
  a.dy = dy; a.x = x; a.ws = ws; a.dy_ldc = (int)g.dy_ldc; a.x_ldc = (int)g.x_ldc;
  a.Hin = g.Hin; a.Win = g.Win; a.Cin = g.Cin; a.Hout = g.Hout; a.Wout = g.Wout; a.Cout = g.Cout;
  a.KH = g.KH; a.KW = g.KW; a.stride = g.stride; a.pad = g.pad; a.dil = g.dil;
  a.M = g.B * g.Hout * g.Wout; a.Ktot = g.KH * g.KW * g.Cin;
  a.pix_per_split = cdiv(cdiv(a.M, splits), bp) * bp;
  a.tiles_k = cdiv(a.Ktot, 128);
  return cdiv(a.M, a.pix_per_split) == splits;
}
unsigned wgrad_grid(WgradArgs& a, int tiles_ck, int splits) {
  a.tiles_ck = tiles_ck;
  a.blocks_total = a.tiles_ck * splits;
  a.xcd_chunk = cdiv(a.blocks_total, 8);
  return (unsigned)(a.xcd_chunk * 8);
}

}

int launch_wgrad_gemm(const WgradGeom& g, const void* dy, const void* x, float* ws, int splits, hipStream_t st) {
  const int dtype = g.dtype;
  WgradArgs a;
  if (!fill_wgrad_args(a, g, dy, x, ws, splits, dtype == MDCV_BF16 ? 128 : 64)) return MDCV_EARG;
  const long long dyb = (long long)a.M * g.dy_ldc * 2, xb = (long long)g.B * g.Hin * g.Win * g.x_ldc * 2;
  const bool use_dma = dtype == MDCV_BF16 && dyb < (1LL << 31) && xb < (1LL << 31) && TUNE().conv_variant != 0 &&
                       (long long)g.B * g.Hin * g.Win + 256 < (1LL << 24) && a.M + 256 < (1 << 24) && g.Wout >= 8 && g.x_ldc < (1 << 23) && g.dy_ldc < (1 << 23);
  const unsigned grid = wgrad_grid(a, a.tiles_k * cdiv(g.Cout, 128), splits);
  const int lds = 256 * (64 * 4 + 16);
  static DynLds dyn_lds16, dyn_lds32;
  if (hipError_t e = mdcv_dyn_lds(dyn_lds16, reinterpret_cast<const void*>(conv_wgrad_kernel<bf16_t>), lds); e != hipSuccess) return (int)e;
  if (hipError_t e = mdcv_dyn_lds(dyn_lds32, reinterpret_cast<const void*>(conv_wgrad_kernel<float>), lds); e != hipSuccess) return (int)e;
  if (use_dma) {
    const int rc = launch_wgrad_dma(a, grid, st, (unsigned)dyb, (unsigned)xb);
    if (rc) return rc;
  } else if (dtype == MDCV_BF16) MDCV_LAUNCH(conv_wgrad_kernel<bf16_t>, dim3(grid), dim3(256), lds, st, a);
  else if (dtype == MDCV_F32) MDCV_LAUNCH(conv_wgrad_kernel<float>, dim3(grid), dim3(256), lds, st, a);
  else return MDCV_EARG;
  MDCV_CHECK_LAUNCH();
  return MDCV_OK;
}

int launch_wgrad_gemm_bnapply(const WgradGeom& g, const void* dz, const void* y, int y_ldc, const float* scale, const float* shift, const float* cA,
                              const float* cB, const float* cC, int act, float slope, int Cout_real, const void* x, float* ws, int splits,
                              hipStream_t st) {
  WgradArgs a;
  if (!fill_wgrad_args(a, g, dz, x, ws, splits, 128)) return MDCV_EARG;
  const unsigned grid = wgrad_grid(a, a.tiles_k, splits);
  a.y = y; a.y_ldc = y_ldc; a.act = act; a.slope = act == 2 ? 0.f : slope; a.creal = Cout_real;
  a.s1 = scale; a.b1 = shift; a.cA = cA; a.cB = cB; a.cC = cC;
  const unsigned dyb = (unsigned)((long long)a.M * g.dy_ldc * 2), xb = (unsigned)((long long)g.B * g.Hin * g.Win * g.x_ldc * 2);
  const bool same = g.stride == 1 && g.Hin == g.Hout && g.Win == g.Wout;
  const int stages = TUNE().wgrad_bna_stages;
  if (stages <= 2) return same ? launch_wgrad_narrow_t<true, 2, true>(a, grid, st, dyb, xb) : launch_wgrad_narrow_t<false, 2, true>(a, grid, st, dyb, xb);
  if (stages == 3) return same ? launch_wgrad_narrow_t<true, 3, true>(a, grid, st, dyb, xb) : launch_wgrad_narrow_t<false, 3, true>(a, grid, st, dyb, xb);
  return same ? launch_wgrad_narrow_t<true, 4, true>(a, grid, st, dyb, xb) : launch_wgrad_narrow_t<false, 4, true>(a, grid, st, dyb, xb);
}
```

mit-driverless-cv-traininginfra_amd/engine.py:

```python
import os

import torch

from . import _lib
from ._lib import F32, BF16, ACT_NONE, ACT_LEAKY, ACT_RELU, tuned


_POISON = os.environ.get("MDCV_POISON", "0") == "1"
_REDZONE = int(os.environ.get("MDCV_REDZONE", "0"))
_RZ_BYTE = 0xA5


def _alloc(n, dtype, device, zero, plan):
    if not _REDZONE:
        t = (torch.zeros if zero else torch.empty)(n, dtype=dtype, device=device)
        if not zero and _POISON and t.is_floating_point():
            t.fill_(float("nan"))
        return t
    es = torch.empty(0, dtype=dtype).element_size()
    raw = torch.full((n * es + _REDZONE,), _RZ_BYTE, dtype=torch.uint8, device=device)
    t = raw[:n * es].view(dtype)
    if zero:
        t.zero_()
    plan.__dict__.setdefault("redzones", []).append((raw, n * es))
    return t


def pad8(c):
    return (c + 7) // 8 * 8


_SIDE_STREAMS = {}


def _runs_beside(others, cand):
    cycles = 1 << 20
    for cur in others:
        e0, e1, e2 = (torch.cuda.Event(enable_timing=True) for _ in range(3))
        with torch.cuda.stream(cur):
            torch.cuda._sleep(cycles)
            cur.synchronize()
            e0.record(cur)
            torch.cuda._sleep(cycles)
            e1.record(cur)
            cand.wait_stream(cur)
            with torch.cuda.stream(cand):
                torch.cuda._sleep(cycles)
            torch.cuda._sleep(cycles)
            cur.wait_stream(cand)
            e2.record(cur)
        e2.synchronize()
        if not e1.elapsed_time(e2) < 1.5 * e0.elapsed_time(e1):
            return False
    return True


def checked_stream(device, beside, key):
    idx = device.index if device.index is not None else torch.cuda.current_device()
    k = (idx, key) + tuple(s.cuda_stream for s in beside)
    s = _SIDE_STREAMS.get(k)
    if s is None:
        if torch.cuda.is_current_stream_capturing():
            return torch.cuda.Stream(device=device)
        ok = False
        with torch.cuda.device(device):
            for _ in range(16):
                s = torch.cuda.Stream(device=device)
                if _runs_beside(beside, s):
                    ok = True
                    break
        if ok:
            _SIDE_STREAMS[k] = s
        else:
            import warnings
            warnings.warn(f"mdcv: no stream of {device} was measured to run beside {key!r}'s partners (16 candidates; busy or shared GPU, "
                          "or too few hardware queues -- GPU_MAX_HW_QUEUES=8 gives HIP more): overlap of this stream is not guaranteed",
                          RuntimeWarning, stacklevel=2)
    return s


def side_stream(device):
    return checked_stream(device, [torch.cuda.current_stream(device)], "side")


def parse_precision(p):
    if p in (BF16, "bf16", torch.bfloat16):
        return BF16
    if p in (F32, "fp32", "f32", torch.float32):
        return F32
    raise ValueError(f"precision must be 'bf16' or 'fp32', got {p!r}")


class Act:
    __slots__ = ("buf", "B", "H", "W", "C", "ldc", "off", "ptr")

    def __init__(self, buf, B, H, W, C, ldc, off=0):
        self.buf, self.B, self.H, self.W, self.C, self.ldc, self.off = buf, B, H, W, C, ldc, off
        self.ptr = buf.data_ptr() + off * buf.element_size()

    @property
    def M(self):
        return self.B * self.H * self.W

    def slice(self, off, C):
        return Act(self.buf, self.B, self.H, self.W, C, self.ldc, self.off + off)

    def dense(self):
        return self.buf.view(self.B, self.H, self.W, self.ldc)[..., self.off:self.off + self.C]


class TNode:
    __slots__ = ("act", "gstate", "grad", "needs_grad", "name")

    def __init__(self, act, needs_grad=True, name=""):
        self.act, self.gstate, self.grad, self.needs_grad, self.name = act, "none", None, needs_grad, name


class ConvSpec:

    def __init__(self, plan, weight, bias, stride, pad, dil, cin_pad=None):
        self.weight, self.bias = weight, bias
        self.cout, self.cin, self.kh, self.kw = weight.shape
        self.stride, self.pad, self.dil = stride, pad, dil
        self.cout_pad = pad8(self.cout)
        self.cin_pad = cin_pad if cin_pad is not None else pad8(self.cin)
        self.ktot = self.kh * self.kw * self.cin_pad
        dt = plan.tdtype
        self.wf = _alloc(self.cout_pad * self.ktot, dt, plan.device, True, plan)
        self.wd = None
        self.bias_pad = None
        if bias is not None:
            self.bias_pad = _alloc(self.cout_pad, torch.float32, plan.device, True, plan)
        plan.keep.append(self)

    def out_hw(self, H, W):
        ek = self.dil * (self.kh - 1) + 1
        return (H + 2 * self.pad - ek) // self.stride + 1, (W + 2 * self.pad - ek) // self.stride + 1


class BnSpec:
    def __init__(self, plan, bn):
        self.bn = bn
        C = bn.num_features
        self.C = C
        dev = plan.device
        z = lambda n=C: _alloc(n, torch.float32, dev, True, plan)
        self.scale, self.shift, self.mean, self.invstd = z(), z(), z(), z()
        self.cA, self.cB, self.cC = z(), z(), z()
        self.accum = _alloc(3 * C, torch.float64, dev, True, plan)
        plan.keep.append(self)


def _variant_env(name):
    raw = (os.environ.get(name) or "0").strip()
    try:
        return int(raw)
    except ValueError:
        raise ValueError(f"{name}={raw!r}: one signed integer variant code per kernel family is carried by every call since round 5 "
                         "(csrc/tune.h lists them); comma-separated lists are no longer accepted") from None


class Plan:
    tune_conv = _variant_env("MDCV_CONV_VARIANT")
    tune_wgrad = _variant_env("MDCV_WGRAD_VARIANT")

    def __init__(self, device, precision, training, grad_sink=None):
        _lib.require_gpu()
        self.L = _lib.lib()
        self.device = device
        self.dtype = parse_precision(precision)
        self.tdtype = torch.bfloat16 if self.dtype == BF16 else torch.float32
        self.cdt = tuned(self.dtype, self.tune_conv)
        self.wdt = tuned(self.dtype, self.tune_wgrad)
        self.training = training
        self.fwd, self.bwd = [], []
        self.keep = []
        self.grad_of = {}
        self.grad_sink = grad_sink
        self.ws_floats = 0
        self._ws = None
        self.bytes = 0
        self.graph_fwd = self.graph_bwd = None
        self.pack_list = []
        self.__dict__.setdefault("redzones", [])
        self.layer_marks = []
        self.param_groups = None
        self._group_events = []
        self._pending_updates = []
        self._packed_ahead = False
        self._packed_version = -1
        self._packed_tversion = -1
        self.owner = None
        self.grad_offset = None
        self.low_water = 1 << 62
        self._last_mark = 1 << 62
        self.on_ready = None
        self.dgrad_entries = {}
        self.fused_bn = 0
        self._fold_candidates = []
        self._xacc_arena, self.stats_xfolded = None, 0

    def new_act(self, B, H, W, C, zero=False):
        Cp = pad8(C)
        buf = _alloc(B * H * W * Cp, self.tdtype, self.device, zero, self)
        self.keep.append(buf)
        self.bytes += buf.numel() * buf.element_size()
        return Act(buf, B, H, W, Cp, Cp)

    def f32(self, n, zero=True):
        t = _alloc(n, torch.float32, self.device, zero, self)
        self.keep.append(t)
        return t

    def param_grad(self, p):
        g = self.grad_of.get(id(p))
        if g is None:
            g = self.grad_sink(p) if self.grad_sink else None
            if g is None:
                g = torch.zeros_like(p, dtype=torch.float32, memory_format=torch.contiguous_format)
            self.grad_of[id(p)] = g
        if self.grad_offset is not None:
            self.low_water = min(self.low_water, self.grad_offset(p))
        return g

    def mark_ready(self):
        lw = self.low_water
        if lw >= self._last_mark:
            return
        self._last_mark = lw
        plan = self

        def ready(stream, lw=lw):
            if plan.on_ready is not None:
                plan.on_ready(lw)
            return 0
        ready.__name__ = "grad_ready"
        ready.low_water = lw
        self.bwd.append((ready, ()))

    def wgrad_ws(self, stream=0):
        if self._ws is None:
            self._ws = {}
        w = self._ws.get(stream)
        if w is None or w.numel() < self.ws_floats:
            w = self._ws[stream] = _alloc(max(self.ws_floats, 1), torch.float32, self.device, False, self)
        return w

    def call(self, lst, fn, *args):
        lst.append((fn, args))

    def run(self, lst, stream=None):
        if stream is None:
            stream = torch.cuda.current_stream().cuda_stream
        for fn, args in lst:
            rc = fn(*args, stream)
            if rc:
                raise _lib.MdcvError(f"{getattr(fn, '__name__', fn)} returned {rc}")

    def grad_target(self, t):
        if t.gstate == "none":
            t.grad = self._alloc_like(t.act)
            t.gstate = "own"
            return t.grad, None
        if t.gstate == "alias":
            src = t.grad
            t.grad = self._alloc_like(t.act)
            t.gstate = "own"
            return t.grad, src
        return t.grad, t.grad

    def grad_identity(self, t, src):
        if not t.needs_grad:
            return
        if t.gstate == "none":
            t.grad, t.gstate = src, "alias"
            return
        if t.gstate == "alias":
            a = t.grad
            t.grad = self._alloc_like(t.act)
            t.gstate = "own"
        else:
            a = t.grad
        self.emit_add(self.bwd, a, src, t.grad)

    def emit_add(self, lst, a, b, out):
        self.call(lst, self.L.bn_act_fwd, self.dtype, a.ptr, a.ldc, None, None, None, 0, None, None, b.ptr if b is not None else None,
                  b.ldc if b is not None else 0, out.ptr, out.ldc, out.M, out.C, ACT_NONE, 0.0)

    def _alloc_like(self, a):
        return self.new_act(a.B, a.H, a.W, a.C)

    def emit_input(self, B, C, H, W):
        a = self.new_act(B, H, W, C)
        node = TNode(a, needs_grad=False, name="input")
        holder = {"src": None}
        L, dt = self.L, self.dtype

        def convert(stream):
            x = holder["src"]
            return L.nchw_to_nhwc(dt, x.data_ptr(), a.ptr, B, C, H, W, a.ldc, a.C, stream)
        convert.__name__ = "nchw_to_nhwc"
        self.fwd.append((convert, ()))
        return node, holder

    def emit_pack(self, cs, need_dgrad):
        if need_dgrad and cs.wd is None:
            cs.wd = _alloc(cs.cin_pad * cs.kh * cs.kw * cs.cout_pad, self.tdtype, self.device, True, self)
        self.pack_list.append(cs)
        self.layer_marks.append(len(self.fwd))

    def stats_rows(self, cs, x, y):
        return int(self.L.conv2d_stats_rows_geom(self.cdt, x.B, y.H, y.W, cs.cin_pad, cs.cout_pad, cs.kh, cs.kw, cs.stride, cs.pad,
                                                 cs.dil, x.ldc))

    def emit_conv_fwd(self, cs, x, y, stats_partial=None):
        assert x.C == cs.cin_pad and y.C == cs.cout_pad, (x.C, cs.cin_pad, y.C, cs.cout_pad)
        self.call(self.fwd, self.L.conv2d, self.cdt, 0, x.ptr, x.ldc, cs.wf.data_ptr(), y.ptr, y.ldc,
                  cs.bias_pad.data_ptr() if cs.bias_pad is not None else None, None, 0,
                  stats_partial.data_ptr() if stats_partial is not None else None,
                  x.B, x.H, x.W, cs.cin_pad, y.H, y.W, cs.cout_pad, cs.kh, cs.kw, cs.stride, cs.pad, cs.dil)

    def emit_conv_bwd(self, cs, xnode, y_shape_act, dy, x_wgrad=None):
        L, dt = self.L, self.dtype
        x = xnode.act
        if x_wgrad is None and self._emit_pw_bwd1(cs, xnode, dy):
            return
        xw = x_wgrad if x_wgrad is not None else x
        cin_w = xw.C if x_wgrad is not None else cs.cin_pad
        if self.wgrad_after_dgrad and cs.kh == 3 and cs.stride == 1:
            self._emit_dgrad(cs, xnode, dy)
            self._emit_wgrad_single(cs, xw, dy, cin_w)
        else:
            self._emit_wgrad_single(cs, xw, dy, cin_w)
            self._emit_dgrad(cs, xnode, dy)

    wgrad_after_dgrad = False

    pw_bwd1 = True

    def _emit_pw_bwd1(self, cs, xnode, dy):
        L, dt = self.L, self.dtype
        x = xnode.act
        if not self.pw_bwd1 or dt != BF16 or not xnode.needs_grad or cs.wd is None:
            return False
        if (cs.kh, cs.kw, cs.stride, cs.pad) != (1, 1, 1, 0) or x.C != cs.cin_pad or dy.C != cs.cout_pad:
            return False
        slabs = int(L.pw_bwd_slabs(dt, x.M, cs.cin_pad, cs.cout_pad, dy.ldc, x.ldc, 8, 8, 8))
        if slabs < 1:
            return False
        out, add = self.grad_target(xnode)
        assert slabs == int(L.pw_bwd_slabs(dt, x.M, cs.cin_pad, cs.cout_pad, dy.ldc, x.ldc, out.ldc, add.ldc if add is not None else 8, 8))
        gw = self.param_grad(cs.weight)
        ws = self.f32(slabs * cs.cout_pad * cs.cin_pad, zero=False)
        args = [dt, dy.ptr, dy.ldc, x.ptr, x.ldc, cs.wd.data_ptr(), out.ptr, out.ldc, add.ptr if add is not None else None,
                add.ldc if add is not None else 0, ws.data_ptr(), slabs, None, 0, None, None, None, 0, 0.0, None, x.M, cs.cin_pad, cs.cout_pad]
        self.dgrad_entries[out.ptr] = dict(
            idx=len(self.bwd), out=out, used=False, pwb=args,
            geom=(x.B, dy.H, dy.W, cs.cout_pad, x.H, x.W, cs.cin_pad, cs.kh, cs.kw, cs.stride, cs.pad, cs.dil), head=(dy.ptr, dy.ldc))
        self.call(self.bwd, L.pw_bwd, *args)

        def wreduce(stream, ws=ws, gw=gw, slabs=slabs, cs=cs):
            return L.wgrad_reduce(ws.data_ptr(), slabs, gw.data_ptr(), 0, cs.cout_pad, cs.cout, cs.cin_pad, cs.cin, 1, stream)
        wreduce.__name__ = "conv2d_wgrad"
        wreduce.info = (x.B, x.H, x.W, cs.cin_pad, dy.H, dy.W, cs.cout_pad, 0, 1, slabs)
        self.bwd.append((wreduce, ()))
        self.pw_bwd1_count = getattr(self, "pw_bwd1_count", 0) + 1
        return True

    def _emit_wgrad_single(self, cs, xw, dy, cin_w):
        L, dt = self.L, self.dtype
        gw = self.param_grad(cs.weight)
        splits = int(L.conv2d_wgrad_splits_geom(self.wdt, xw.B, xw.H, xw.W, cin_w, dy.H, dy.W, cs.cout_pad, cs.kh, cs.kw, cs.stride, cs.pad,
                                                cs.dil, dy.ldc, xw.ldc))
        self.ws_floats = max(self.ws_floats, splits * cs.cout_pad * cs.kh * cs.kw * cin_w)
        plan = self

        def wgrad(stream, cs=cs, x=xw, dy=dy, gw=gw, splits=splits, cin_w=cin_w):
            return L.conv2d_wgrad(plan.wdt, dy.ptr, dy.ldc, x.ptr, x.ldc, plan.wgrad_ws(stream).data_ptr(), splits, gw.data_ptr(), 0,
                                  x.B, x.H, x.W, cin_w, cs.cin, dy.H, dy.W, cs.cout_pad, cs.cout, cs.kh, cs.kw,
                                  cs.stride, cs.pad, cs.dil, stream)
        wgrad.__name__ = "conv2d_wgrad"
        wgrad.info = (xw.B, xw.H, xw.W, cin_w, dy.H, dy.W, cs.cout_pad, cs.kh, cs.stride, splits)
        self.bwd.append((wgrad, ()))

    def _emit_dgrad(self, cs, xnode, dy):
        L, dt = self.L, self.dtype
        x = xnode.act
        if xnode.needs_grad:
            out, add = self.grad_target(xnode)
            self.dgrad_entries[out.ptr] = dict(
                idx=len(self.bwd), out=out, used=False,
                geom=(x.B, dy.H, dy.W, cs.cout_pad, x.H, x.W, cs.cin_pad, cs.kh, cs.kw, cs.stride, cs.pad, cs.dil),
                head=(dy.ptr, dy.ldc, cs.wd.data_ptr(), out.ptr, out.ldc, add.ptr if add is not None else None,
                      add.ldc if add is not None else 0))
            self.call(self.bwd, L.conv2d, self.cdt, 1, dy.ptr, dy.ldc, cs.wd.data_ptr(), out.ptr, out.ldc, None,
                      add.ptr if add is not None else None, add.ldc if add is not None else 0, None,
                      x.B, dy.H, dy.W, cs.cout_pad, x.H, x.W, cs.cin_pad, cs.kh, cs.kw, cs.stride, cs.pad, cs.dil)

    def emit_bias_grad(self, cs, dy, zero_only=False):
        gb = self.param_grad(cs.bias)
        if zero_only:
            gb.zero_()
            return
        tmp = self.f32(cs.cout_pad)
        pws = self.f32(int(self.L.colsum_ws_floats(self.dtype, dy.M, cs.cout_pad)), zero=False)
        self.call(self.bwd, self.L.colsum_f32, self.dtype, dy.ptr, dy.ldc, dy.M, cs.cout_pad, pws.data_ptr(), tmp.data_ptr())

        def copy(stream, gb=gb, tmp=tmp, n=cs.cout):
            gb.copy_(tmp[:n].view_as(gb), non_blocking=True)
            return 0
        copy.__name__ = "copy_bias_grad"
        self.bwd.append((copy, ()))

    def emit_bn_stats(self, bs, y, partial, rows):
        L = self.L
        bn = bs.bn
        self.call(self.fwd, L.bn_stats_finalize, partial.data_ptr(), rows, bs.accum.data_ptr(), float(y.M), bn.weight.data_ptr(),
                  bn.bias.data_ptr(), bn.running_mean.data_ptr(), bn.running_var.data_ptr(), float(bn.momentum), float(bn.eps),
                  bs.scale.data_ptr(), bs.shift.data_ptr(), bs.mean.data_ptr(), bs.invstd.data_ptr(), bs.C)

    def emit_bn_eval(self, bs):
        bn = bs.bn
        self.call(self.fwd, self.L.bn_eval_coeffs, bn.weight.data_ptr(), bn.bias.data_ptr(), bn.running_mean.data_ptr(),
                  bn.running_var.data_ptr(), float(bn.eps), bs.scale.data_ptr(), bs.shift.data_ptr(), bs.C)

    def emit_conv_bn_act_eval(self, cs, bs, x, out, act, slope, resid=None):
        bn = bs.bn
        self.call(self.fwd, self.L.bn_eval_coeffs_bias, bn.weight.data_ptr(), bn.bias.data_ptr(), bn.running_mean.data_ptr(),
                  bn.running_var.data_ptr(), float(bn.eps), cs.bias_pad.data_ptr() if cs.bias_pad is not None else None,
                  bs.scale.data_ptr(), bs.shift.data_ptr(), bs.C)
        self.call(self.fwd, self.L.conv2d_affine_act, self.cdt, x.ptr, x.ldc, cs.wf.data_ptr(), out.ptr, out.ldc, bs.scale.data_ptr(),
                  bs.shift.data_ptr(), resid.ptr if resid is not None else None, resid.ldc if resid is not None else 0, act, float(slope),
                  x.B, x.H, x.W, cs.cin_pad, out.H, out.W, cs.cout_pad, cs.kh, cs.kw, cs.stride, cs.pad, cs.dil)

    def emit_bn_act_fwd(self, y1, bs1, out, act, slope, y2=None, bs2=None, resid=None):
        self.last_bnact = None if y2 is not None else dict(idx=len(self.fwd), y=y1, bs=bs1, out=out, act=act, slope=float(slope), resid=resid)
        self.call(self.fwd, self.L.bn_act_fwd, self.dtype, y1.ptr, y1.ldc, bs1.scale.data_ptr(), bs1.shift.data_ptr(),
                  y2.ptr if y2 is not None else None, y2.ldc if y2 is not None else 0,
                  bs2.scale.data_ptr() if bs2 is not None else None, bs2.shift.data_ptr() if bs2 is not None else None,
                  resid.ptr if resid is not None else None, resid.ldc if resid is not None else 0,
                  out.ptr, out.ldc, out.M, out.C, act, float(slope))

    def note_stats_fold(self, conv, fin, act, cs, x, y, bs, partial, rows, out, act_code, slope, resid):
        self._fold_candidates.append((conv, fin, act, cs, x, y, bs, partial, rows, out, act_code, float(slope), resid))

    stats_xacc = True
    stats_xacc_pw = True
    stats_xacc_words = 1 << 20
    stats_xacc_chain = 1024

    def fold_forward_xstats(self):
        L, dt = self.L, self.dtype
        if not self.stats_xacc or self._xacc_arena is None:
            return 0
        cands, self._fold_candidates = self._fold_candidates, []
        arena = self._xacc_arena
        used, done = 0, 0
        for conv, fin, act, cs, x, y, bs, partial, rows, out, act_code, slope, resid in cands:
            idx = [i for i, e in enumerate(self.fwd) if e is conv]
            if len(idx) != 1:
                continue
            i = idx[0]
            if i + 2 > len(self.fwd) - 1 or self.fwd[i + 1] is not fin:
                continue
            nxt = self.fwd[i + 2]
            pw_next = (self.stats_xacc_pw and nxt is not act and nxt[0] in (L.pw_conv_fwd, L.pw_conv_fwd_xstats) and len(nxt[1]) > 4
                       and nxt[1][3] == bs.scale.data_ptr() and nxt[1][1] == y.ptr)
            if nxt is not act and not pw_next:
                continue
            if y.C > 1024:
                continue
            reps = int(L.xstats_reps(rows, y.C))
            if rows > self.stats_xacc_chain * reps:
                continue
            need = int(L.xstats_words(reps, y.C))
            if used + need > arena.numel():
                continue
            acc = arena[used:used + need]
            used += need
            bn = bs.bn
            a = conv[1]
            if conv[0] is L.pw_conv_fwd:
                self.fwd[i] = (L.pw_conv_fwd_xstats, a[:15] + (acc.data_ptr(), reps) + a[16:])
            elif conv[0] is L.conv2d:
                self.fwd[i] = (L.conv2d_xstats, (a[0],) + a[2:8] + (acc.data_ptr(), reps) + a[11:])
            else:
                used -= need
                continue
            if pw_next:
                self.fwd[i + 1] = (L.bn_act_fwd_xstats, (dt, y.ptr, y.ldc, acc.data_ptr(), reps, float(y.M), bn.weight.data_ptr(), bn.bias.data_ptr(),
                                                         bn.running_mean.data_ptr(), bn.running_var.data_ptr(), float(bn.momentum), float(bn.eps),
                                                         bs.scale.data_ptr(), bs.shift.data_ptr(), bs.mean.data_ptr(), bs.invstd.data_ptr(),
                                                         None, 0, y.ptr, y.ldc, 0, y.C, act_code, slope))
                done += 1
                continue
            self.fwd[i + 2] = (L.bn_act_fwd_xstats, (dt, y.ptr, y.ldc, acc.data_ptr(), reps, float(y.M), bn.weight.data_ptr(), bn.bias.data_ptr(),
                                                     bn.running_mean.data_ptr(), bn.running_var.data_ptr(), float(bn.momentum), float(bn.eps),
                                                     bs.scale.data_ptr(), bs.shift.data_ptr(), bs.mean.data_ptr(), bs.invstd.data_ptr(),
                                                     resid.ptr if resid is not None else None, resid.ldc if resid is not None else 0,
                                                     out.ptr, out.ldc, out.M, out.C, act_code, slope))
            del self.fwd[i + 1]
            self.layer_marks = [m - 1 if m > i + 1 else m for m in self.layer_marks]
            done += 1
        for k, e in enumerate(self.fwd):
            if len(e[1]) == 1 and e[1][0] is arena:
                view = arena[:max(used, 1)]
                self.keep.append(view)
                self.fwd[k] = (e[0], (view,))
                break
        self.stats_xfolded = done
        return done

    pw_fuse = True
    pw_fwd_px = (50000, 1 << 30)

    def _pw_ok(self, cs, M, K, N, *lds):
        if not self.pw_fuse or self.dtype != BF16 or not self.training:
            return False
        if (cs.kh, cs.kw, cs.stride, cs.pad) != (1, 1, 1, 0):
            return False
        lo, hi = self.pw_fwd_px
        if not (lo <= M < hi) or N < 64:
            return False
        if K > 512:
            return False
        if K < 64 or K % 32 or 256 % (K // 8) or N % 8 or any(v % 8 for v in lds):
            return False
        return True

    def pw_fwd_candidate(self, cs_shape, x):
        lb = getattr(self, "last_bnact", None)
        if lb is None or lb["idx"] != len(self.fwd) - 1 or lb["out"].ptr != x.ptr or lb["out"].ldc != x.ldc or lb["out"].C != x.C:
            return None
        cout, cin, kh, kw, stride, pad = cs_shape

        class _S:
            pass
        c = _S(); c.kh, c.kw, c.stride, c.pad = kh, kw, stride, pad
        r = lb["resid"]
        if not self._pw_ok(c, x.M, x.C, pad8(cout), lb["y"].ldc, x.ldc, r.ldc if r is not None else 8):
            return None
        return lb

    def emit_pw_fwd(self, lb, cs, x, y, stats_partial):
        assert lb["idx"] == len(self.fwd) and x.C == cs.cin_pad and y.C == cs.cout_pad
        self.last_bnact = None
        r, bs = lb["resid"], lb["bs"]
        self.call(self.fwd, self.L.pw_conv_fwd, self.dtype, lb["y"].ptr, lb["y"].ldc, bs.scale.data_ptr(), bs.shift.data_ptr(),
                  r.ptr if r is not None else None, r.ldc if r is not None else 0, lb["act"], lb["slope"], x.ptr, x.ldc,
                  cs.wf.data_ptr(), cs.bias_pad.data_ptr() if cs.bias_pad is not None else None, y.ptr, y.ldc,
                  stats_partial.data_ptr() if stats_partial is not None else None, x.M, cs.cin_pad, cs.cout_pad)
        self.pw_fwd_count = getattr(self, "pw_fwd_count", 0) + 1

    def emit_bn_act_bwd(self, dout, y1, bs1, act, slope, y2=None, bs2=None, apply=True):
        L, dt = self.L, self.dtype
        dy1 = self._alloc_like(y1) if apply else None
        dy2 = self._alloc_like(y2) if y2 is not None else None
        n = lambda t: t.data_ptr() if t is not None else None
        pws = self.f32(L.bn_act_bwd_reduce_ws_floats(dt, y1.M, y1.C, 3 if y2 is not None else 2), zero=False)
        g1, b1 = self.param_grad(bs1.bn.weight), self.param_grad(bs1.bn.bias)
        g2 = b2 = None
        if y2 is not None:
            g2, b2 = self.param_grad(bs2.bn.weight), self.param_grad(bs2.bn.bias)
        fused = y2 is None and self._fuse_bn_sums(dout, y1, bs1, act, slope, g1, b1)
        if not fused:
            self.call(self.bwd, L.bn_act_bwd_reduce_finalize, dt, dout.ptr, dout.ldc, y1.ptr, y1.ldc, n(bs1.scale), n(bs1.shift), n(bs1.mean),
                      n(bs1.invstd), y2.ptr if y2 is not None else None, y2.ldc if y2 is not None else 0,
                      n(bs2.scale) if bs2 else None, n(bs2.shift) if bs2 else None, n(bs2.mean) if bs2 else None,
                      n(bs2.invstd) if bs2 else None, pws.data_ptr(), y1.M, y1.C, act, float(slope), float(y1.M),
                      bs1.bn.weight.data_ptr(), g1.data_ptr(), b1.data_ptr(), n(bs1.cA), n(bs1.cB), n(bs1.cC),
                      bs2.bn.weight.data_ptr() if bs2 else None, n(g2), n(b2), n(bs2.cA) if bs2 else None, n(bs2.cB) if bs2 else None,
                      n(bs2.cC) if bs2 else None)
        if not apply:
            assert y2 is None
            return None
        self.call(self.bwd, L.bn_act_bwd_apply, dt, dout.ptr, dout.ldc, y1.ptr, y1.ldc, n(bs1.scale), n(bs1.shift), n(bs1.cA),
                  n(bs1.cB), n(bs1.cC), dy1.ptr, dy1.ldc,
                  y2.ptr if y2 is not None else None, y2.ldc if y2 is not None else 0,
                  n(bs2.scale) if bs2 else None, n(bs2.shift) if bs2 else None, n(bs2.cA) if bs2 else None,
                  n(bs2.cB) if bs2 else None, n(bs2.cC) if bs2 else None,
                  dy2.ptr if dy2 is not None else None, dy2.ldc if dy2 is not None else 0, y1.M, y1.C, act, float(slope))
        return (dy1, dy2) if y2 is not None else dy1

    wgrad_bnapply = True
    first_conv_2pass = True

    def emit_first_conv_bwd(self, dout, y, bs, act, slope, cs, xnode):
        L = self.L
        x = xnode.act
        if not self.wgrad_bnapply or xnode.needs_grad or self.dtype != BF16 or cs.bias is not None:
            return False
        geom = (x.B, x.H, x.W, cs.cin_pad, y.H, y.W, cs.cout_pad, cs.kh, cs.kw, cs.stride, cs.pad, cs.dil)
        if not int(L.conv2d_wgrad_bnapply_ok(self.wdt, *geom, dout.ldc, y.ldc, x.ldc)):
            return False
        self.emit_bn_act_bwd(dout, y, bs, act, slope, apply=False)
        gw = self.param_grad(cs.weight)
        sdt = _lib.tuned(self.dtype, 20000 + 768) if self.tune_wgrad == 0 else self.wdt
        splits = int(L.conv2d_wgrad_splits_geom(sdt, *geom, dout.ldc, x.ldc))
        self.ws_floats = max(self.ws_floats, splits * cs.cout_pad * cs.kh * cs.kw * cs.cin_pad)
        plan = self
        n = lambda t: t.data_ptr()

        def wgrad(stream):
            return L.conv2d_wgrad_bnapply(plan.wdt, dout.ptr, dout.ldc, y.ptr, y.ldc, n(bs.scale), n(bs.shift), n(bs.cA), n(bs.cB), n(bs.cC), act,
                                          float(slope), x.ptr, x.ldc, plan.wgrad_ws(stream).data_ptr(), splits, gw.data_ptr(), 0, x.B, x.H, x.W,
                                          cs.cin_pad, cs.cin, y.H, y.W, cs.cout_pad, cs.cout, cs.kh, cs.kw, cs.stride, cs.pad, cs.dil, stream)
        wgrad.__name__ = "conv2d_wgrad"
        wgrad.info = (x.B, x.H, x.W, cs.cin_pad, y.H, y.W, cs.cout_pad, cs.kh, cs.stride, splits)
        self.bwd.append((wgrad, ()))
        self.first_conv_fused = True
        return True

    fuse_bn = True

    fuse_skip = 141
    fuse_max_rows = 4096
    fuse_max_rows_s2 = 1 << 16

    def _fuse_pays(self, geom):
        B, dyH, dyW, cdy, xH, xW, cdx, kh, kw, stride, pad, dil = geom
        px = B * xH * xW
        k = self.fuse_skip
        if kh == 3 and stride == 1:
            if 50000 <= px < 100000:
                return not (k & 1)
            if 20000 <= px < 50000:
                return not (k & 2)
            if px >= 300000:
                return not (k & 32)
            if px < 20000:
                return not (k & 256)
        if kh == 1:
            if px >= 300000:
                return not (k & 4)
            if 50000 <= px < 100000:
                return not (k & 16)
            if 20000 <= px < 50000:
                return not (k & 64)
            if px < 20000:
                return not (k & 512)
        if stride == 2 and 300000 <= px < 1000000:
            return not (k & 8)
        if stride == 2 and px < 300000:
            return not (k & 128)
        return True

    def _fuse_bn_sums(self, dout, y, bs, act, slope, dgamma, dbeta):
        if not self.fuse_bn or self.dtype != BF16:
            return False
        e = self.dgrad_entries.get(dout.ptr)
        if e is None or e["used"]:
            return False
        o = e["out"]
        if (o.M, o.C, o.ldc) != (dout.M, dout.C, dout.ldc) or (y.M, y.C) != (dout.M, dout.C):
            return False
        for fn, args in self.bwd[e["idx"] + 1:]:
            if dout.ptr in args:
                return False
        L, dt = self.L, self.dtype
        pwb = e.get("pwb")
        g = e["geom"]
        if pwb is not None:
            rows = int(pwb[11])
            partial = self.f32(rows * 2 * y.C, zero=False)
            a2 = list(pwb)
            a2[12:20] = [y.ptr, y.ldc, bs.scale.data_ptr(), bs.shift.data_ptr(), bs.mean.data_ptr(), act, float(slope), partial.data_ptr()]
            assert self.bwd[e["idx"]][0] is L.pw_bwd
            self.bwd[e["idx"]] = (L.pw_bwd, tuple(a2))
        else:
            s2_shift = bool(L.conv2d_dgrad_s2_form_ok(self.cdt, *g, e["head"][1]))
            if not s2_shift and not self._fuse_pays(g):
                return False
            rows = int(L.conv2d_dgrad_bnsums_rows(self.cdt, *g, e["head"][1]))
            if rows <= 0 or rows > (self.fuse_max_rows_s2 if s2_shift else self.fuse_max_rows):
                return False
            assert self.bwd[e["idx"]][0] is L.conv2d
            partial = self.f32(rows * 2 * y.C, zero=False)
            h = e["head"]
            self.bwd[e["idx"]] = (L.conv2d_dgrad_bnsums, (self.cdt, h[0], h[1], h[2], h[3], h[4], h[5], h[6], *e["geom"], y.ptr, y.ldc,
                                                          bs.scale.data_ptr(), bs.shift.data_ptr(), bs.mean.data_ptr(), act, float(slope),
                                                          partial.data_ptr()))
        e["used"] = True
        self.call(self.bwd, L.bn_bwd_finalize_rows, partial.data_ptr(), rows, y.C, float(y.M), bs.bn.weight.data_ptr(),
                  bs.mean.data_ptr(), bs.invstd.data_ptr(), dgamma.data_ptr(), dbeta.data_ptr(), bs.cA.data_ptr(), bs.cB.data_ptr(),
                  bs.cC.data_ptr())
        self.fused_bn += 1
        return True

    def finish_pack(self, position=0):
        import struct
        rec = b"".join(struct.pack("<QQQiiiiiiiiQQ", cs.weight.data_ptr(), cs.wf.data_ptr(), cs.wd.data_ptr() if cs.wd is not None else 0,
                                   cs.cout, cs.cin, cs.kh * cs.kw, cs.cout_pad, cs.cin_pad, 0, 0, 0,
                                   cs.bias.data_ptr() if cs.bias is not None else 0,
                                   cs.bias_pad.data_ptr() if cs.bias is not None else 0) for cs in self.pack_list)
        table = torch.frombuffer(bytearray(rec), dtype=torch.uint8).to(self.device)
        self.keep.append(table)
        eq_taps = max(1, max((min(64, cs.cin_pad) * cs.kh * cs.kw + 63) // 64 for cs in self.pack_list))
        self.pack_table, self.pack_eq_taps = table, eq_taps
        plan = self
        args = (self.dtype, table.data_ptr(), len(self.pack_list), eq_taps)

        def pack_all(stream):
            owner = plan.owner
            if plan._packed_ahead:
                plan._packed_ahead = False
                if owner is None or (getattr(owner, "_param_epoch", 0) == plan._packed_version
                                     and owner._param_versions() == plan._packed_tversion):
                    return 0
            if owner is not None:
                owner._param_sync()
            return plan.L.pack_weights_batched(*args, stream)
        pack_all.__name__ = "mdcv_pack_weights_batched"
        self.fwd.insert(position, (pack_all, ()))
        self.layer_marks = [m + 1 if m >= position else m for m in self.layer_marks]

    def check_redzones(self):
        bad = 0
        for raw, n in self.redzones:
            if int((raw[n:] != _RZ_BYTE).sum()):
                bad += 1
        return bad

    def launch_param_group(self, k, gated):
        if 0 <= k < len(self._pending_updates) and self._pending_updates[k] is not None:
            fn, self._pending_updates[k] = self._pending_updates[k], None
            fn(torch.cuda.current_stream() if gated else None)

    def ensure_param_groups(self, pflat):
        if self.param_groups is not None:
            return self.param_groups
        self.param_groups = []
        base, n = pflat.data_ptr(), pflat.numel()
        offs = [(cs.weight.data_ptr() - base) // 4 for cs in self.pack_list]
        if not offs or any(o < 0 or o >= n for o in offs) or any(b <= a for a, b in zip(offs, offs[1:])):
            return self.param_groups
        firsts, target, lo = [0], 128 * 1024, 0
        for li in range(1, len(offs)):
            if offs[li] - lo >= target:
                firsts.append(li)
                lo = offs[li]
                target = min(target * 4, 12 * 1024 * 1024)
        groups = []
        for gi, f in enumerate(firsts):
            last = firsts[gi + 1] if gi + 1 < len(firsts) else len(offs)
            groups.append((0 if gi == 0 else offs[f], offs[last] if last < len(offs) else n, f, last - f))
        self._group_events = [None] * len(groups)
        self._pending_updates = [None] * len(groups)
        plan = self
        for k in range(len(groups) - 1, -1, -1):
            def wait_params(stream, k=k):
                plan.launch_param_group(k, gated=False)
                ev = plan._group_events[k]
                if ev is not None:
                    torch.cuda.current_stream().wait_event(ev)
                    plan._group_events[k] = None
                plan.launch_param_group(k + 2, gated=True)
                return 0
            wait_params.__name__ = "wait_params"
            self.fwd.insert(self.layer_marks[groups[k][2]], (wait_params, ()))
        self.param_groups = groups
        return groups

    def capture(self, which, stream=None):
        L = self.L
        if stream is None:
            stream = torch.cuda.current_stream().cuda_stream
        lst = self.fwd if which == "fwd" else self.bwd
        import ctypes
        L.check(L.graph_begin(stream), "graph_begin")
        try:
            self.run(lst, stream)
        finally:
            ge = ctypes.c_void_p()
            rc = L.graph_end(stream, ctypes.byref(ge))
        L.check(rc, "graph_end")
        return ge


def run_timed(plan, lst, stream=None, kernels=False):
    import ctypes
    L = plan.L
    if stream is None:
        stream = torch.cuda.current_stream().cuda_stream
    evs = []
    for _ in range(len(lst) + 1):
        e = ctypes.c_void_p()
        L.check(L.event_create(ctypes.byref(e)), "event_create")
        evs.append(e)
    spans = []
    if kernels:
        L.check(L.profile_begin(), "profile_begin")
    L.check(L.event_record(evs[0], stream))
    try:
        for i, (fn, args) in enumerate(lst):
            n0 = L.profile_count() if kernels else 0
            rc = fn(*args, stream)
            if rc:
                raise _lib.MdcvError(f"{getattr(fn, '__name__', fn)} returned {rc}")
            spans.append((n0, L.profile_count() if kernels else 0))
            L.check(L.event_record(evs[i + 1], stream))
    finally:
        nrec = L.profile_stop() if kernels else 0
    L.check(L.event_sync(evs[-1]))
    krec = []
    if kernels:
        if nrec < 0:
            raise _lib.MdcvError(f"mdcv_profile_stop failed ({nrec})")
        buf = ctypes.create_string_buffer(1024)
        for i in range(nrec):
            ms = ctypes.c_float()
            L.check(L.profile_read(i, ctypes.byref(ms), buf, 1024), "profile_read")
            krec.append((buf.value.decode(), ms.value))
    out = []
    for i, (fn, args) in enumerate(lst):
        ms = ctypes.c_float()
        L.check(L.event_elapsed_ms(evs[i], evs[i + 1], ctypes.byref(ms)))
        ent = (getattr(fn, "__name__", str(fn)), ms.value, args if args else getattr(fn, "info", ()))
        out.append(ent + (krec[spans[i][0]:spans[i][1]],) if kernels else ent)
    for e in evs:
        L.event_destroy(e)
    return out
```

Measured before the change: 2465 images/sec.

## Recompute first conv output in backward instead of storing pre-BN activation

For the first 3x3 conv (Cin=8, Cout=32), the forward pass no longer writes the pre-BN output y. Backward recomputes it on the fly from x and the forward weights with MFMA, once in a new kernel that produces the BN backward sums and again inside the fused wgrad+BN-apply kernel. This cuts a large full-resolution activation write and two reads from HBM at 416x416. The cost is extra conv arithmetic in two backward kernels and added code complexity.

```diff
diff --git a/include/mdcv_hip.h b/include/mdcv_hip.h
--- a/include/mdcv_hip.h
+++ b/include/mdcv_hip.h
@@ -31,6 +31,10 @@
 int mdcv_first_conv_stats(int dtype, const void* x, int ldx, const void* w_packed, float* partial, int B, int H, int W, void* stream);
 int mdcv_first_conv_bn_act(int dtype, const void* x, int ldx, const void* w_packed, const float* scale, const float* shift, int act, float slope,
                            void* y, int ldy, void* z, int ldz, int B, int H, int W, void* stream);
+int mdcv_first_conv_bwd_sums_ok(int dtype, int B, int H, int W, int Cin_pad, int Cout_pad, int KH, int KW, int stride, int pad, int dil, int ldx, int lddz);
+int mdcv_first_conv_bwd_sums_rows(int B, int H);
+int mdcv_first_conv_bwd_sums(int dtype, const void* x, int ldx, const void* w_packed, const void* dz, int lddz, const float* scale, const float* shift,
+                             const float* mean, int act, float slope, float* partial, int B, int H, int W, void* stream);
 int mdcv_conv2d_dgrad_s2_form_ok(int dtype, int B, int Hin, int Win, int Cin, int Hout, int Wout, int Nout, int KH, int KW, int stride,
                                  int pad, int dil, int in_ldc);
 int mdcv_xstats_words(int reps, int C);
@@ -247,6 +251,12 @@
                               const float* cA, const float* cB, const float* cC, int act, float slope, const void* x, int x_ldc, float* ws,
                               int splits, float* dw_oihw, int accumulate, int B, int Hin, int Win, int Cin, int Cin_real, int Hout, int Wout,
                               int Cout, int Cout_real, int KH, int KW, int stride, int pad, int dil, void* stream);
+int mdcv_conv2d_wgrad_bnapply_x_ok(int dtype, int B, int Hin, int Win, int Cin, int Hout, int Wout, int Cout, int KH, int KW, int stride,
+                                   int pad, int dil, int dz_ldc, int x_ldc);
+int mdcv_conv2d_wgrad_bnapply_x(int dtype, const void* dz, int dz_ldc, const void* w_fwd, const float* scale, const float* shift,
+                                const float* cA, const float* cB, const float* cC, int act, float slope, const void* x, int x_ldc, float* ws,
+                                int splits, float* dw_oihw, int accumulate, int B, int Hin, int Win, int Cin, int Cin_real, int Hout, int Wout,
+                                int Cout, int Cout_real, int KH, int KW, int stride, int pad, int dil, void* stream);
 int mdcv_wgrad_reduce(const float* ws, int splits, float* dw_oihw, int accumulate, int Cout_pad, int Cout, int Cin_pad, int Cin, int KK,
                       void* stream);
 
diff --git a/mit-driverless-cv-traininginfra_amd/csrc/conv_igemm.hip b/mit-driverless-cv-traininginfra_amd/csrc/conv_igemm.hip
--- a/mit-driverless-cv-traininginfra_amd/csrc/conv_igemm.hip
+++ b/mit-driverless-cv-traininginfra_amd/csrc/conv_igemm.hip
@@ -279,9 +279,27 @@
   if (!dz || !y || !scale || !shift || !cA || !cB || !cC || !x || !ws || !dw_oihw || splits < 1) return MDCV_EARG;
   if (!mdcv_conv2d_wgrad_bnapply_ok(dtype, B, Hin, Win, Cin, Hout, Wout, Cout, KH, KW, stride, pad, dil, dz_ldc, y_ldc, x_ldc)) return MDCV_EARG;
   const WgradGeom g{dtype, B, Hin, Win, Cin, Hout, Wout, Cout, KH, KW, stride, pad, dil, dz_ldc, x_ldc};
-  const int rc = launch_wgrad_gemm_bnapply(g, dz, y, y_ldc, scale, shift, cA, cB, cC, act, slope, Cout_real, x, ws, splits, (hipStream_t)stream);
+  const int rc = launch_wgrad_gemm_bnapply(g, dz, y, nullptr, y_ldc, scale, shift, cA, cB, cC, act, slope, Cout_real, x, ws, splits, (hipStream_t)stream);
   if (rc) return rc;
   return launch_wgrad_reduce(ws, dw_oihw, splits, Cout, Cout_real, Cin, Cin_real, KH * KW, accumulate, (hipStream_t)stream);
 }
 
-}
+int mdcv_conv2d_wgrad_bnapply_x_ok(int dtype, int B, int Hin, int Win, int Cin, int Hout, int Wout, int Cout, int KH, int KW, int stride,
+                                   int pad, int dil, int dz_ldc, int x_ldc) {
+  return Cin == 8 && x_ldc == 8 && Cout == 32 && KH == 3 && KW == 3 && stride == 1 && pad == 1 && dil == 1 && Hin == Hout && Win == Wout &&
+         mdcv_conv2d_wgrad_bnapply_ok(dtype, B, Hin, Win, Cin, Hout, Wout, Cout, KH, KW, stride, pad, dil, dz_ldc, Cout, x_ldc);
+}
+int mdcv_conv2d_wgrad_bnapply_x(int dtype, const void* dz, int dz_ldc, const void* w_fwd, const float* scale, const float* shift,
+                                const float* cA, const float* cB, const float* cC, int act, float slope, const void* x, int x_ldc, float* ws,
+                                int splits, float* dw_oihw, int accumulate, int B, int Hin, int Win, int Cin, int Cin_real, int Hout, int Wout,
+                                int Cout, int Cout_real, int KH, int KW, int stride, int pad, int dil, void* stream) {
+  MDCV_TUNE_ENTRY(dtype, MDCV_TUNE_WGRAD);
+  if (!dz || !w_fwd || !scale || !shift || !cA || !cB || !cC || !x || !ws || !dw_oihw || splits < 1) return MDCV_EARG;
+  if (!mdcv_conv2d_wgrad_bnapply_x_ok(dtype, B, Hin, Win, Cin, Hout, Wout, Cout, KH, KW, stride, pad, dil, dz_ldc, x_ldc)) return MDCV_EARG;
+  const WgradGeom g{dtype, B, Hin, Win, Cin, Hout, Wout, Cout, KH, KW, stride, pad, dil, dz_ldc, x_ldc};
+  const int rc = launch_wgrad_gemm_bnapply(g, dz, nullptr, w_fwd, Cout, scale, shift, cA, cB, cC, act, slope, Cout_real, x, ws, splits, (hipStream_t)stream);
+  if (rc) return rc;
+  return launch_wgrad_reduce(ws, dw_oihw, splits, Cout, Cout_real, Cin, Cin_real, KH * KW, accumulate, (hipStream_t)stream);
+}
+
+}
diff --git a/mit-driverless-cv-traininginfra_amd/csrc/first_conv.hip b/mit-driverless-cv-traininginfra_amd/csrc/first_conv.hip
--- a/mit-driverless-cv-traininginfra_amd/csrc/first_conv.hip
+++ b/mit-driverless-cv-traininginfra_amd/csrc/first_conv.hip
@@ -10,7 +10,8 @@
   const bf16_t* x; const bf16_t* wf;
   bf16_t* y; bf16_t* z; const float* scale; const float* shift;
   float* partial;
-  int ldx, ldy, ldz, B, H, W, strips, act;
+  const bf16_t* dz; const float* mean;
+  int ldx, ldy, ldz, lddz, B, H, W, strips, act;
   float slope;
 };
 
@@ -53,7 +54,8 @@
     for (int s = 0; s < 3; ++s) {
       const int tap = 4 * s + kg;
       uint4 v = make_uint4(0u, 0u, 0u, 0u);
-      if (tap < 9) v = *reinterpret_cast<const uint4*>(a.wf + ((size_t)(h * 16 + l16) * 9 + tap) * CIN);
+      const int co = MODE == 2 ? (l16 >> 2) * 8 + h * 4 + (l16 & 3) : h * 16 + l16;
+      if (tap < 9) v = *reinterpret_cast<const uint4*>(a.wf + ((size_t)co * 9 + tap) * CIN);
       wa[h][s] = __builtin_bit_cast(bf16x8_t, v);
     }
   int boff[3];
@@ -64,12 +66,21 @@
     const int dy = tap / 3, dx = tap - dy * 3;
     boff[s] = (dy * WP + l16 + dx) * PXB;
   }
-  float sc[2][4], sh[2][4];
-  if constexpr (MODE == 1) {
+  float sc[2][4], sh[2][4], mn[2][4];
+  if constexpr (MODE == 1 || MODE == 3) {
 #pragma unroll
     for (int h = 0; h < 2; ++h)
 #pragma unroll
       for (int r = 0; r < 4; ++r) { sc[h][r] = a.scale[h * 16 + kg * 4 + r]; sh[h][r] = a.shift[h * 16 + kg * 4 + r]; }
+  }
+  if constexpr (MODE == 2) {
+#pragma unroll
+    for (int h = 0; h < 2; ++h)
+#pragma unroll
+      for (int r = 0; r < 4; ++r) {
+        const int c = kg * 8 + h * 4 + r;
+        sc[h][r] = a.scale[c]; sh[h][r] = a.shift[c]; mn[h][r] = a.mean[c];
+      }
   }
   float ssum[2][4], ssq[2][4];
 #pragma unroll
@@ -77,6 +88,95 @@
 #pragma unroll
     for (int r = 0; r < 4; ++r) { ssum[h][r] = 0.f; ssq[h][r] = 0.f; }
   __syncthreads();
+
+  float sg[2][4], sx[2][4];
+  if constexpr (MODE == 2) {
+    constexpr int DQ = 4;
+#pragma unroll
+    for (int h = 0; h < 2; ++h)
+#pragma unroll
+      for (int r = 0; r < 4; ++r) { sg[h][r] = 0.f; sx[h][r] = 0.f; }
+    for (int lr = wave; lr < TR; lr += NW) {
+      const int row = r0 + lr;
+      if (row >= a.H) break;
+      const bf16_t* const dzr = a.dz + ((size_t)img * a.H + row) * a.W * a.lddz + kg * 8;
+      const unsigned char* const rb = smem + (size_t)lr * WP * PXB;
+      const int clast = (a.W - 1) & ~15;
+      auto load_dz = [&](int c0) {
+        const int px = c0 + l16 < a.W ? c0 + l16 : a.W - 1;
+        return *reinterpret_cast<const uint4*>(dzr + (size_t)px * a.lddz);
+      };
+      uint4 dq[DQ];
+#pragma unroll
+      for (int u = 0; u < DQ; ++u) dq[u] = load_dz(u * 16);
+      uint4 bn[3];
+#pragma unroll
+      for (int s = 0; s < 3; ++s) bn[s] = *reinterpret_cast<const uint4*>(rb + boff[s]);
+      for (int cq = 0; cq < a.W; cq += 16 * DQ) {
+#pragma unroll
+        for (int u = 0; u < DQ; ++u) {
+          const int c0 = cq + u * 16;
+          uint4 b[3];
+#pragma unroll
+          for (int s = 0; s < 3; ++s) b[s] = bn[s];
+          const int cn = c0 + 16 < clast ? c0 + 16 : clast;
+#pragma unroll
+          for (int s = 0; s < 3; ++s) bn[s] = *reinterpret_cast<const uint4*>(rb + boff[s] + cn * PXB);
+          f32x4_t acc[2] = {{0.f, 0.f, 0.f, 0.f}, {0.f, 0.f, 0.f, 0.f}};
+#pragma unroll
+          for (int s = 0; s < 3; ++s) {
+            const bf16x8_t bb = __builtin_bit_cast(bf16x8_t, b[s]);
+            acc[0] = __builtin_amdgcn_mfma_f32_16x16x32_bf16(wa[0][s], bb, acc[0], 0, 0, 0);
+            acc[1] = __builtin_amdgcn_mfma_f32_16x16x32_bf16(wa[1][s], bb, acc[1], 0, 0, 0);
+          }
+          float dv[8];
+          ET<bf16_t>::unpack(dq[u], dv);
+          dq[u] = load_dz(c0 + 16 * DQ);
+          const bool live = c0 + l16 < a.W;
+#pragma unroll
+          for (int h = 0; h < 2; ++h) {
+            uint2 yq;
+            yq.x = pack_bf16x2(acc[h][0], acc[h][1]); yq.y = pack_bf16x2(acc[h][2], acc[h][3]);
+            float v[4];
+            v[0] = __uint_as_float(yq.x << 16); v[1] = __uint_as_float(yq.x & 0xffff0000u);
+            v[2] = __uint_as_float(yq.y << 16); v[3] = __uint_as_float(yq.y & 0xffff0000u);
+#pragma unroll
+            for (int r = 0; r < 4; ++r) {
+              const float pre = __builtin_fmaf(v[r], sc[h][r], sh[h][r]);
+              const float d = dv[h * 4 + r];
+              const float g = (a.act != 0 && !(pre > 0.f)) ? d * a.slope : d;
+              sg[h][r] += live ? g : 0.f;
+              sx[h][r] += live ? g * (v[r] - mn[h][r]) : 0.f;
+            }
+          }
+        }
+      }
+    }
+#pragma unroll
+    for (int h = 0; h < 2; ++h)
+#pragma unroll
+      for (int r = 0; r < 4; ++r)
+#pragma unroll
+        for (int o = 8; o >= 1; o >>= 1) { sg[h][r] += __shfl_xor(sg[h][r], o, 64); sx[h][r] += __shfl_xor(sx[h][r], o, 64); }
+    float* red = reinterpret_cast<float*>(stage);
+    if (l16 == 0) {
+#pragma unroll
+      for (int h = 0; h < 2; ++h)
+#pragma unroll
+        for (int r = 0; r < 4; ++r) {
+          red[(wave * 2 + 0) * COUT + kg * 8 + h * 4 + r] = sg[h][r];
+          red[(wave * 2 + 1) * COUT + kg * 8 + h * 4 + r] = sx[h][r];
+        }
+    }
+    __syncthreads();
+    if (tid < 2 * COUT) {
+      float t = 0.f;
+#pragma unroll
+      for (int w = 0; w < NW; ++w) t += red[w * 2 * COUT + tid];
+      a.partial[(size_t)blockIdx.x * 2 * COUT + tid] = t;
+    }
+    return;
+  }
 
   unsigned char* const st = stage + wave * 2048;
   for (int lr = wave; lr < TR; lr += NW) {
@@ -123,16 +223,17 @@
             v[r] = a.act == 0 ? pre : (pre > 0.f ? pre : pre * a.slope);
           }
           zq.x = pack_bf16x2(v[0], v[1]); zq.y = pack_bf16x2(v[2], v[3]);
-          *reinterpret_cast<uint2*>(st + l16 * 64 + (h * 16 + kg * 4) * 2) = yq;
+          if constexpr (MODE == 1) *reinterpret_cast<uint2*>(st + l16 * 64 + (h * 16 + kg * 4) * 2) = yq;
           *reinterpret_cast<uint2*>(st + 1024 + l16 * 64 + (h * 16 + kg * 4) * 2) = zq;
         }
         asm volatile("s_waitcnt lgkmcnt(0)" ::: "memory");
-        const uint4 yo = *reinterpret_cast<const uint4*>(st + lane * 16);
+        uint4 yo = make_uint4(0u, 0u, 0u, 0u);
+        if constexpr (MODE == 1) yo = *reinterpret_cast<const uint4*>(st + lane * 16);
         const uint4 zo = *reinterpret_cast<const uint4*>(st + 1024 + lane * 16);
         asm volatile("s_waitcnt lgkmcnt(0)" ::: "memory");
         const int px = c0 + (lane >> 2);
         if (px < a.W) {
-          *reinterpret_cast<uint4*>(a.y + (rowpix + px) * a.ldy + (lane & 3) * 8) = yo;
+          if constexpr (MODE == 1) *reinterpret_cast<uint4*>(a.y + (rowpix + px) * a.ldy + (lane & 3) * 8) = yo;
           *reinterpret_cast<uint4*>(a.z + (rowpix + px) * a.ldz + (lane & 3) * 8) = zo;
         }
       }
@@ -193,7 +294,7 @@
 
 int mdcv_first_conv_bn_act(int dtype, const void* x, int ldx, const void* w_packed, const float* scale, const float* shift, int act, float slope,
                            void* y, int ldy, void* z, int ldz, int B, int H, int W, void* stream) {
-  if (!x || !w_packed || !scale || !shift || !y || !z || (ldy & 7) || (ldz & 7) || ldy < COUT || ldz < COUT ||
+  if (!x || !w_packed || !scale || !shift || !z || (y && ((ldy & 7) || ldy < COUT)) || (ldz & 7) || ldz < COUT ||
       !mdcv_first_conv_ok(dtype, B, H, W, CIN, COUT, 3, 3, 1, 1, 1, ldx))
     return MDCV_EARG;
   FirstConvArgs a{};
@@ -201,11 +302,40 @@
   a.y = reinterpret_cast<bf16_t*>(y); a.z = reinterpret_cast<bf16_t*>(z); a.scale = scale; a.shift = shift;
   a.ldx = ldx; a.ldy = ldy; a.ldz = ldz; a.B = B; a.H = H; a.W = W; a.strips = nstrips(H); a.act = act; a.slope = act == 2 ? 0.f : slope;
   const int lds = (int)lds_bytes(W);
-  static DynLds dyn;
+  static DynLds dyn, dynz;
+  if (!y) {
+    if (hipError_t e = mdcv_dyn_lds(dynz, reinterpret_cast<const void*>(first_conv_kernel<3>), lds); e != hipSuccess) return (int)e;
+    MDCV_LAUNCH(first_conv_kernel<3>, dim3((unsigned)(B * a.strips)), dim3(NW * 64), lds, (hipStream_t)stream, a);
+    MDCV_CHECK_LAUNCH();
+    return MDCV_OK;
+  }
   if (hipError_t e = mdcv_dyn_lds(dyn, reinterpret_cast<const void*>(first_conv_kernel<1>), lds); e != hipSuccess) return (int)e;
   MDCV_LAUNCH(first_conv_kernel<1>, dim3((unsigned)(B * a.strips)), dim3(NW * 64), lds, (hipStream_t)stream, a);
   MDCV_CHECK_LAUNCH();
   return MDCV_OK;
 }
 
-}
+int mdcv_first_conv_bwd_sums_ok(int dtype, int B, int H, int W, int Cin_pad, int Cout_pad, int KH, int KW, int stride, int pad, int dil, int ldx, int lddz) {
+  return mdcv_first_conv_ok(dtype, B, H, W, Cin_pad, Cout_pad, KH, KW, stride, pad, dil, ldx) && !(lddz & 7) && lddz >= COUT &&
+         (long long)B * H * W * lddz * 2 < (1LL << 40);
+}
+int mdcv_first_conv_bwd_sums_rows(int B, int H) { return B * nstrips(H); }
+
+int mdcv_first_conv_bwd_sums(int dtype, const void* x, int ldx, const void* w_packed, const void* dz, int lddz, const float* scale, const float* shift,
+                             const float* mean, int act, float slope, float* partial, int B, int H, int W, void* stream) {
+  if (!x || !w_packed || !dz || !scale || !shift || !mean || !partial ||
+      !mdcv_first_conv_bwd_sums_ok(dtype, B, H, W, CIN, COUT, 3, 3, 1, 1, 1, ldx, lddz))
+    return MDCV_EARG;
+  FirstConvArgs a{};
+  a.x = reinterpret_cast<const bf16_t*>(x); a.wf = reinterpret_cast<const bf16_t*>(w_packed); a.dz = reinterpret_cast<const bf16_t*>(dz);
+  a.scale = scale; a.shift = shift; a.mean = mean; a.partial = partial;
+  a.ldx = ldx; a.lddz = lddz; a.B = B; a.H = H; a.W = W; a.strips = nstrips(H); a.act = act; a.slope = act == 2 ? 0.f : slope;
+  const int lds = (int)lds_bytes(W);
+  static DynLds dyn;
+  if (hipError_t e = mdcv_dyn_lds(dyn, reinterpret_cast<const void*>(first_conv_kernel<2>), lds); e != hipSuccess) return (int)e;
+  MDCV_LAUNCH(first_conv_kernel<2>, dim3((unsigned)(B * a.strips)), dim3(NW * 64), lds, (hipStream_t)stream, a);
+  MDCV_CHECK_LAUNCH();
+  return MDCV_OK;
+}
+
+}
diff --git a/mit-driverless-cv-traininginfra_amd/csrc/wgrad_gemm.h b/mit-driverless-cv-traininginfra_amd/csrc/wgrad_gemm.h
--- a/mit-driverless-cv-traininginfra_amd/csrc/wgrad_gemm.h
+++ b/mit-driverless-cv-traininginfra_amd/csrc/wgrad_gemm.h
@@ -7,7 +7,7 @@
 };
 
 int launch_wgrad_gemm(const WgradGeom& g, const void* dy, const void* x, float* ws, int splits, hipStream_t st);
-int launch_wgrad_gemm_bnapply(const WgradGeom& g, const void* dz, const void* y, int y_ldc, const float* scale, const float* shift, const float* cA,
+int launch_wgrad_gemm_bnapply(const WgradGeom& g, const void* dz, const void* y, const void* w_fwd, int y_ldc, const float* scale, const float* shift, const float* cA,
                               const float* cB, const float* cC, int act, float slope, int Cout_real, const void* x, float* ws, int splits,
                               hipStream_t st);
 int launch_wgrad_reduce(const float* ws, float* dw_oihw, int splits, int Cout_pad, int Cout_real, int Cin_pad, int Cin_real, int KK, int accumulate,
diff --git a/mit-driverless-cv-traininginfra_amd/csrc/wgrad_gemm.hip b/mit-driverless-cv-traininginfra_amd/csrc/wgrad_gemm.hip
--- a/mit-driverless-cv-traininginfra_amd/csrc/wgrad_gemm.hip
+++ b/mit-driverless-cv-traininginfra_amd/csrc/wgrad_gemm.hip
@@ -11,6 +11,7 @@
   int M, Ktot, tiles_k, tiles_ck, pix_per_split, blocks_total, xcd_chunk;
   const void* y; int y_ldc, act, creal; float slope;
   const float* s1; const float* b1; const float* cA; const float* cB; const float* cC;
+  const void* wfwd;
 };
 
 template <typename T>
@@ -340,10 +341,11 @@
   }
 }
 
-template <bool SAME, int STAGES, bool BNA = false>
+template <bool SAME, int STAGES, bool BNA = false, bool YF = false>
 __global__ __launch_bounds__(256) void conv_wgrad_dma_narrow_kernel(WgradArgs a, unsigned dy_bytes, unsigned x_bytes) {
-  constexpr int BP = 64, NJ = 4, GD = BNA ? 6 : 5;
-  constexpr int TA = BP * 64 * (BNA ? 2 : 1), TB = BP * 256;
+  static_assert(!YF || (BNA && SAME), "the y-free form is a BNA form of same-size layers");
+  constexpr int BP = 64, NJ = 4, GD = (BNA && !YF) ? 6 : 5;
+  constexpr int TA = BP * 64 * ((BNA && !YF) ? 2 : 1), TB = BP * 256;
   constexpr int OROW = 132;
   constexpr unsigned OOB = 0x80000000u;
   extern __shared__ __attribute__((aligned(1024))) unsigned char smem[];
@@ -388,7 +390,7 @@
       const int m = m0 + 16 * wave + ra;
       const unsigned offa = (m < p_end && a_ok) ? __umul24((unsigned)m, ldy2) + (unsigned)coA * 2u : OOB;
       __builtin_amdgcn_raw_ptr_buffer_load_lds(rdy, (lds_void_t*)(sA + wave * 1024), 16, offa, 0, 0, 0);
-      if constexpr (BNA) {
+      if constexpr (BNA && !YF) {
         const unsigned offy = (m < p_end && a_ok) ? __umul24((unsigned)m, (unsigned)a.y_ldc * 2u) + (unsigned)coA * 2u : OOB;
         __builtin_amdgcn_raw_ptr_buffer_load_lds(ry, (lds_void_t*)(sA + BP * 64 + wave * 1024), 16, offy, 0, 0, 0);
       }
@@ -476,6 +478,73 @@
     const uint4 qo = ET<bf16_t>::pack(o);
     const u32x4_t wo = {qo.x, qo.y, qo.z, qo.w};
     asm volatile("ds_write_b128 %0, %1" ::"v"(ad), "v"(wo) : "memory");
+  };
+
+  bf16x8_t wy[YF ? 2 : 1][YF ? 3 : 1];
+  unsigned yrd[YF ? 3 : 1], ydz[YF ? 2 : 1];
+  float ys1[YF ? 8 : 1], yb1[YF ? 8 : 1], yA[YF ? 8 : 1], yB[YF ? 8 : 1], yC[YF ? 8 : 1];
+  const int pY = 16 * wave + t;
+  if constexpr (YF) {
+#pragma unroll
+    for (int s = 0; s < 3; ++s) {
+      const int tap = 4 * s + kq;
+#pragma unroll
+      for (int h = 0; h < 2; ++h) {
+        uint4 v = make_uint4(0u, 0u, 0u, 0u);
+        if (tap < 9) v = *reinterpret_cast<const uint4*>(reinterpret_cast<const bf16_t*>(a.wfwd) + ((size_t)(h * 16 + t) * 9 + tap) * 8);
+        wy[h][s] = __builtin_bit_cast(bf16x8_t, v);
+      }
+      const int tp = tap < 9 ? tap : 8;
+      yrd[s] = (unsigned)(TA + pY * 256 + ((tp ^ (2 * (pY & 7))) << 4));
+    }
+#pragma unroll
+    for (int h = 0; h < 2; ++h) {
+      ydz[h] = (unsigned)(pY * 64 + (((2 * h + (kq >> 1)) ^ (2 * ((pY >> 2) & 1))) << 4) + (kq & 1) * 8);
+#pragma unroll
+      for (int r = 0; r < 4; ++r) {
+        const int c = 16 * h + 4 * kq + r, e = 4 * h + r;
+        const bool ok = c < a.creal;
+        ys1[e] = ok ? a.s1[c] : 0.f; yb1[e] = ok ? a.b1[c] : 0.f;
+        yA[e] = ok ? a.cA[c] : 0.f; yB[e] = ok ? a.cB[c] : 0.f; yC[e] = ok ? a.cC[c] : 0.f;
+      }
+    }
+  }
+  auto transform_y = [&](int slot, int m0) {
+   if constexpr (YF) {
+    const unsigned base = lds_addr(smem + slot * (TA + TB));
+    typedef unsigned u32x4_t __attribute__((ext_vector_type(4)));
+    typedef unsigned u32x2_t __attribute__((ext_vector_type(2)));
+    u32x4_t xb[3];
+    u32x2_t dq[2];
+#pragma unroll
+    for (int s = 0; s < 3; ++s) asm volatile("ds_read_b128 %0, %1" : "=v"(xb[s]) : "v"(base + yrd[s]) : "memory");
+#pragma unroll
+    for (int h = 0; h < 2; ++h) asm volatile("ds_read_b64 %0, %1" : "=v"(dq[h]) : "v"(base + ydz[h]) : "memory");
+    asm volatile("s_waitcnt lgkmcnt(0)" : "+v"(xb[0]), "+v"(xb[1]), "+v"(xb[2]), "+v"(dq[0]), "+v"(dq[1])::"memory");
+    f32x4_t ya[2] = {{0.f, 0.f, 0.f, 0.f}, {0.f, 0.f, 0.f, 0.f}};
+#pragma unroll
+    for (int s = 0; s < 3; ++s) {
+      const bf16x8_t bb = __builtin_bit_cast(bf16x8_t, xb[s]);
+      ya[0] = __builtin_amdgcn_mfma_f32_16x16x32_bf16(wy[0][s], bb, ya[0], 0, 0, 0);
+      ya[1] = __builtin_amdgcn_mfma_f32_16x16x32_bf16(wy[1][s], bb, ya[1], 0, 0, 0);
+    }
+    const bool live = m0 + pY < p_end;
+#pragma unroll
+    for (int h = 0; h < 2; ++h) {
+      const unsigned y0 = pack_bf16x2(ya[h][0], ya[h][1]), y1 = pack_bf16x2(ya[h][2], ya[h][3]);
+      const float v[4] = {__uint_as_float(y0 << 16), __uint_as_float(y0 & 0xffff0000u), __uint_as_float(y1 << 16), __uint_as_float(y1 & 0xffff0000u)};
+      const float d[4] = {__uint_as_float(dq[h][0] << 16), __uint_as_float(dq[h][0] & 0xffff0000u), __uint_as_float(dq[h][1] << 16),
+                          __uint_as_float(dq[h][1] & 0xffff0000u)};
+      float o[4];
+#pragma unroll
+      for (int r = 0; r < 4; ++r) {
+        const int e = 4 * h + r;
+        o[r] = live ? mdcv_bn_bwd_dy(d[r], v[r], ys1[e], yb1[e], yA[e], yB[e], yC[e], a.act, a.slope) : 0.f;
+      }
+      const u32x2_t wo = {pack_bf16x2(o[0], o[1]), pack_bf16x2(o[2], o[3])};
+      asm volatile("ds_write_b64 %0, %1" ::"v"(base + ydz[h]), "v"(wo) : "memory");
+    }
+   }
   };
 
   f32x4_t acc[2][2];
@@ -518,7 +587,8 @@
       islot = islot + 1 == STAGES ? 0 : islot + 1;
     }
     if constexpr (BNA) {
-      transform(slot, p_begin + st * BP);
+      if constexpr (YF) transform_y(slot, p_begin + st * BP);
+      else transform(slot, p_begin + st * BP);
       asm volatile("s_waitcnt lgkmcnt(0)" ::: "memory");
       __builtin_amdgcn_s_barrier();
     }
@@ -556,11 +626,11 @@
   MDCV_CHECK_LAUNCH();
   return MDCV_OK;
 }
-template <bool SAME, int STAGES, bool BNA = false>
+template <bool SAME, int STAGES, bool BNA = false, bool YF = false>
 static int launch_wgrad_narrow_t(const WgradArgs& a, unsigned grid, hipStream_t st, unsigned dyb, unsigned xb) {
-  constexpr int LDS = STAGES * (64 * 64 * (BNA ? 2 : 1) + 64 * 256);
+  constexpr int LDS = STAGES * (64 * 64 * ((BNA && !YF) ? 2 : 1) + 64 * 256);
   static DynLds dyn_lds;
-  auto kern = conv_wgrad_dma_narrow_kernel<SAME, STAGES, BNA>;
+  auto kern = conv_wgrad_dma_narrow_kernel<SAME, STAGES, BNA, YF>;
   if (hipError_t e = mdcv_dyn_lds(dyn_lds, reinterpret_cast<const void*>(kern), LDS); e != hipSuccess) return (int)e;
   MDCV_LAUNCH(kern, dim3(grid), dim3(256), LDS, st, a, dyb, xb);
   MDCV_CHECK_LAUNCH();
@@ -614,17 +684,23 @@
   return MDCV_OK;
 }
 
-int launch_wgrad_gemm_bnapply(const WgradGeom& g, const void* dz, const void* y, int y_ldc, const float* scale, const float* shift, const float* cA,
+int launch_wgrad_gemm_bnapply(const WgradGeom& g, const void* dz, const void* y, const void* w_fwd, int y_ldc, const float* scale, const float* shift, const float* cA,
                               const float* cB, const float* cC, int act, float slope, int Cout_real, const void* x, float* ws, int splits,
                               hipStream_t st) {
   WgradArgs a;
   if (!fill_wgrad_args(a, g, dz, x, ws, splits, 128)) return MDCV_EARG;
   const unsigned grid = wgrad_grid(a, a.tiles_k, splits);
   a.y = y; a.y_ldc = y_ldc; a.act = act; a.slope = act == 2 ? 0.f : slope; a.creal = Cout_real;
-  a.s1 = scale; a.b1 = shift; a.cA = cA; a.cB = cB; a.cC = cC;
+  a.s1 = scale; a.b1 = shift; a.cA = cA; a.cB = cB; a.cC = cC; a.wfwd = w_fwd;
   const unsigned dyb = (unsigned)((long long)a.M * g.dy_ldc * 2), xb = (unsigned)((long long)g.B * g.Hin * g.Win * g.x_ldc * 2);
   const bool same = g.stride == 1 && g.Hin == g.Hout && g.Win == g.Wout;
   const int stages = TUNE().wgrad_bna_stages;
+  if (!y) {
+    if (!w_fwd || !same || a.tiles_k != 1) return MDCV_EARG;
+    if (stages <= 2) return launch_wgrad_narrow_t<true, 2, true, true>(a, grid, st, dyb, xb);
+    if (stages == 3) return launch_wgrad_narrow_t<true, 3, true, true>(a, grid, st, dyb, xb);
+    return launch_wgrad_narrow_t<true, 4, true, true>(a, grid, st, dyb, xb);
+  }
   if (stages <= 2) return same ? launch_wgrad_narrow_t<true, 2, true>(a, grid, st, dyb, xb) : launch_wgrad_narrow_t<false, 2, true>(a, grid, st, dyb, xb);
   if (stages == 3) return same ? launch_wgrad_narrow_t<true, 3, true>(a, grid, st, dyb, xb) : launch_wgrad_narrow_t<false, 3, true>(a, grid, st, dyb, xb);
   return same ? launch_wgrad_narrow_t<true, 4, true>(a, grid, st, dyb, xb) : launch_wgrad_narrow_t<false, 4, true>(a, grid, st, dyb, xb);
diff --git a/mit-driverless-cv-traininginfra_amd/engine.py b/mit-driverless-cv-traininginfra_amd/engine.py
--- a/mit-driverless-cv-traininginfra_amd/engine.py
+++ b/mit-driverless-cv-traininginfra_amd/engine.py
@@ -585,6 +585,22 @@
     wgrad_bnapply = True
     first_conv_2pass = True
 
+    first_conv_recompute = True
+    first_conv_recompute_parts = 3
+
+    def _first_conv_recompute(self, dout, y, cs, x, geom):
+        L = self.L
+        parts = self.first_conv_recompute_parts if self.first_conv_recompute else 0
+        idx = next((i for i, (fn, args) in enumerate(self.fwd) if fn is L.first_conv_bn_act and args[8] == y.ptr), None)
+        if not parts or idx is None or not self.training:
+            return False, False, None
+        sums = bool(parts & 1) and bool(L.first_conv_bwd_sums_ok(self.dtype, x.B, x.H, x.W, cs.cin_pad, cs.cout_pad, cs.kh, cs.kw, cs.stride, cs.pad,
+                                                                cs.dil, x.ldc, dout.ldc))
+        wfree = bool(parts & 2) and bool(L.conv2d_wgrad_bnapply_x_ok(self.wdt, *geom, dout.ldc, x.ldc))
+        if self.first_conv_recompute_parts == 3 and not (sums and wfree):
+            return False, False, None
+        return sums, wfree, idx
+
     def emit_first_conv_bwd(self, dout, y, bs, act, slope, cs, xnode):
         L = self.L
         x = xnode.act
@@ -593,15 +609,32 @@
         geom = (x.B, x.H, x.W, cs.cin_pad, y.H, y.W, cs.cout_pad, cs.kh, cs.kw, cs.stride, cs.pad, cs.dil)
         if not int(L.conv2d_wgrad_bnapply_ok(self.wdt, *geom, dout.ldc, y.ldc, x.ldc)):
             return False
-        self.emit_bn_act_bwd(dout, y, bs, act, slope, apply=False)
+        n = lambda t: t.data_ptr()
+        sums, wfree, fidx = self._first_conv_recompute(dout, y, cs, x, geom)
+        if sums:
+            dgamma, dbeta = self.param_grad(bs.bn.weight), self.param_grad(bs.bn.bias)
+            rows = int(L.first_conv_bwd_sums_rows(x.B, x.H))
+            partial = self.f32(rows * 2 * y.C, zero=False)
+            self.call(self.bwd, L.first_conv_bwd_sums, self.dtype, x.ptr, x.ldc, cs.wf.data_ptr(), dout.ptr, dout.ldc, n(bs.scale), n(bs.shift),
+                      n(bs.mean), act, float(slope), partial.data_ptr(), x.B, x.H, x.W)
+            self.call(self.bwd, L.bn_bwd_finalize_rows, partial.data_ptr(), rows, y.C, float(y.M), n(bs.bn.weight), n(bs.mean), n(bs.invstd),
+                      n(dgamma), n(dbeta), n(bs.cA), n(bs.cB), n(bs.cC))
+        else:
+            self.emit_bn_act_bwd(dout, y, bs, act, slope, apply=False)
+        if sums and wfree:
+            fn, a = self.fwd[fidx]
+            self.fwd[fidx] = (fn, a[:8] + (None, 0) + a[10:])
         gw = self.param_grad(cs.weight)
         sdt = _lib.tuned(self.dtype, 20000 + 768) if self.tune_wgrad == 0 else self.wdt
         splits = int(L.conv2d_wgrad_splits_geom(sdt, *geom, dout.ldc, x.ldc))
         self.ws_floats = max(self.ws_floats, splits * cs.cout_pad * cs.kh * cs.kw * cs.cin_pad)
         plan = self
-        n = lambda t: t.data_ptr()
 
         def wgrad(stream):
+            if wfree:
+                return L.conv2d_wgrad_bnapply_x(plan.wdt, dout.ptr, dout.ldc, cs.wf.data_ptr(), n(bs.scale), n(bs.shift), n(bs.cA), n(bs.cB), n(bs.cC),
+                                                act, float(slope), x.ptr, x.ldc, plan.wgrad_ws(stream).data_ptr(), splits, gw.data_ptr(), 0, x.B, x.H,
+                                                x.W, cs.cin_pad, cs.cin, y.H, y.W, cs.cout_pad, cs.cout, cs.kh, cs.kw, cs.stride, cs.pad, cs.dil, stream)
             return L.conv2d_wgrad_bnapply(plan.wdt, dout.ptr, dout.ldc, y.ptr, y.ldc, n(bs.scale), n(bs.shift), n(bs.cA), n(bs.cB), n(bs.cC), act,
                                           float(slope), x.ptr, x.ldc, plan.wgrad_ws(stream).data_ptr(), splits, gw.data_ptr(), 0, x.B, x.H, x.W,
                                           cs.cin_pad, cs.cin, y.H, y.W, cs.cout_pad, cs.cout, cs.kh, cs.kw, cs.stride, cs.pad, cs.dil, stream)
@@ -609,6 +642,7 @@
         wgrad.info = (x.B, x.H, x.W, cs.cin_pad, y.H, y.W, cs.cout_pad, cs.kh, cs.stride, splits)
         self.bwd.append((wgrad, ()))
         self.first_conv_fused = True
+        self.first_conv_recomputed = (sums, wfree)
         return True
 
     fuse_bn = True
```

Result: no change. 2484 images/sec, median of 6 (+0.7%).
